# pearsonlab/autoencoded-vocal-analysis

Hardware: AMD Instinct MI355X
Metric: spectrograms/sec, VAE train step (fwd+bwd+Adam), 128x128, batch 256 per GPU (higher is better)
Workload: dtype f32 (fc1/fc8 products, the forward convolutions with >= 8 input channels and the fused backward kernels (data gradient AND weight gradient): fp32 operands as three bf16 limbs on bf16 MFMA, six limb products, fp32 accumulate; the 1<->8-channel layers, convt6's forward, conv7's forward and the small f; 1 GPU; configs[1]: mouse_sylls VAE, batch 256 synthetic 128x128 fp32 spectrograms per GPU, z=32, train step = zero_grad+forward+backward+Adam, device-resident batches; global_batch=256, per_gpu_batch=256, z_dim=32, parallelism=dp1

## Files before the change

autoencoded-vocal-analysis_amd/_lib.py:

```python
import ctypes as C
import os
import subprocess

_HERE = os.path.dirname(os.path.abspath(__file__))
CSRC = os.path.join(_HERE, "csrc")
_TAG = os.environ.get("AVA_HIP_LIB_TAG", "")
LIB_PATH = os.path.join(CSRC, "libava_hip_%s.so" % _TAG if _TAG else "libava_hip.so")

_ERR = {-1: "AVA_EINVAL (bad argument / unsupported shape)", -2: "AVA_ELAUNCH (HIP launch failure)",
        -3: "AVA_EWORKSPACE (workspace too small)"}


class AvaHipError(RuntimeError):
    pass


def build(force=False, verbose=False):
    cmd = ["make", "-C", CSRC, "-j8"] + (["-B"] if force else [])
    res = subprocess.run(cmd, capture_output=True, text=True)
    if verbose or res.returncode != 0:
        print(res.stdout)
        print(res.stderr)
    if res.returncode != 0:
        raise AvaHipError("building libava_hip.so failed")
    return LIB_PATH


_p = C.c_void_p
_i = C.c_int
_i64 = C.c_int64
_f = C.c_float
_d = C.c_double
_sz = C.c_size_t

SIGNATURES = {
    "ava_version": (_i, []),
    "ava_arena_floats": (_i64, [_i]),
    "ava_param_offset": (_i64, [_i, _i, C.POINTER(_i64)]),
    "ava_workspace_bytes": (_sz, [_i, _i]),
    "ava_model_create": (_i, [C.POINTER(_p), _i, _i, _f, _p, _p, _p, _p, _p, _p, _p, _sz]),
    "ava_model_destroy": (None, [_p]),
    "ava_arena_floats_hw": (_i64, [_i, _i, _i]),
    "ava_param_offset_hw": (_i64, [_i, _i, _i, _i, C.POINTER(_i64)]),
    "ava_workspace_bytes_hw": (_sz, [_i, _i, _i, _i]),
    "ava_model_create_hw": (_i, [C.POINTER(_p), _i, _i, _i, _i, _f, _p, _p, _p, _p, _p, _p, _p, _sz]),
    "ava_model_create_ex": (_i, [C.POINTER(_p), _i, _i, _i, _i, _i, _f, _p, _p, _p, _p, _p, _p, _p, _sz]),
    "ava_forward": (_i, [_p, _p, _i, _p, _p, _i, _p, _p, _p, _p]),
    "ava_forward_noise": (_i, [_p, _p, _i, _p, C.c_uint64, C.c_uint64, _i, _p, _p, _p, _p]),
    "ava_backward": (_i, [_p, _p, _i, _p]),
    "ava_set_backward_scale": (_i, [_p, _p]),
    "ava_backward_num_parts": (_i, []),
    "ava_backward_part": (_i, [_p, _p, _i, _i, _p]),
    "ava_grad_bucket": (_i, [_p, _i, C.POINTER(_i64), C.POINTER(_i64)]),
    "ava_adam_step": (_i, [_p, _d, _d, _d, _d, _i, _p]),
    "ava_adam_step_range": (_i, [_p, _i64, _i64, _d, _d, _d, _d, _i, _p]),
    "ava_encode": (_i, [_p, _p, _i, _i, _p, _p, _p, _p]),
    "ava_decode": (_i, [_p, _p, _i, _i, _p, _p]),
    "ava_last_z": (_p, [_p]),
    "ava_last_xrec": (_p, [_p]),
    "ava_debug_buffer": (_p, [_p, C.c_char_p, C.POINTER(_i64)]),
    "ava_debug_materialize": (_i, [_p, _p, _i, _p]),
    "ava_set_cu_reserve": (_i, [_i]),
    "ava_get_cu_reserve": (_i, []),
    "ava_model_set_cu_reserve": (_i, [_p, _i]),
    "ava_model_get_cu_reserve": (_i, [_p]),
    "ava_occupy_cus": (_i, [_i, _i, _f, _p]),
    "ava_profile_enable": (_i, [_p, _i]),
    "ava_profile_read": (_i, [_p, C.POINTER(_f), C.POINTER(_i)]),
    "ava_fill_normal": (_i, [_p, _i64, C.c_uint64, C.c_uint64, _p]),
    "ava_pack_conv_weight": (_i, [_p, _p, _i, _i, _i, _p]),
    "ava_conv_grid": (_i, [_i, _i, _i, _i]),
    "ava_conv3x3": (_i, [_p] * 13 + [_i] * 9 + [_f, _p]),
    "ava_conv3x3_wgrad": (_i, [_p] * 9 + [_i] * 7 + [_p]),
    "ava_conv_wgrad_grid": (_i, [_i, _i, _i, _i]),
    "ava_conv_wgrad_rows": (_i, [_i, _i, _i, _i, _i, _i, _i]),
    "ava_conv_fused_grid": (_i, [_i, _i, _i, _i, _i, _i]),
    "ava_conv3x3_bwd_fused": (_i, [_p] * 14 + [_i] * 7 + [_p]),
    "ava_conv_wgrad_reduce": (_i, [_p, _i, _p, _p, _i, _i, _i, _p]),
    "ava_bn_stats": (_i, [_p, _i64, _i, _p, C.POINTER(_i), _p]),
    "ava_bn_finalize": (_i, [_p, _i, _i64, _i, _p, _p, _p, _p, _p, _i, _p, _p, _p, _p, _p]),
    "ava_bn_finalize_bwd": (_i, [_p, _i, _i64, _i, _p, _p, _p, _p, _p, _p, _p, _p, _p]),
    "ava_gemm_workspace_bytes": (_sz, [_i, _i, _i]),
    "ava_gemm": (_i, [_p, _i, _p, _i, _p, _p, _i, _p, _p, _i, _i, _i, _i, _i, _i, _p, _sz, _p]),
    "ava_latent_fwd": (_i, [_p] * 9 + [_i, _i, _p]),
    "ava_latent_bwd": (_i, [_p] * 9 + [_i, _i, _p]),
    "ava_elbo_finalize": (_i, [_p, _i, _p, _i, _i, _f, _p, _p]),
    "ava_adam_flat": (_i, [_p, _p, _p, _p, _i64, _d, _d, _d, _d, _i, _p]),
    "ava_cast_to_f32": (_i, [_p, _i, _i64, _p, _p]),
    "ava_host_gather_rows": (_i, [_p, _p, _p, _i64, _i64, _sz, _i]),
    "ava_mmd2_workspace_bytes": (_sz, [_i, _i]),
    "ava_mmd2": (_i, [_p, _i, _p, _i, _p, _i, _d, _p, _p, _sz, _p]),
    "ava_mmd2_linear": (_i, [_p, _i, _p, _p, _i, _d, _p, _p, _sz, _p]),
    "ava_pair_sqdist": (_i, [_p, _i, _p, _p, _i, _p, _p]),
    "ava_spec_workspace_bytes": (_sz, [_i, _i, _i, _i, _i, _i, _i]),
    "ava_get_spec_batch": (_i, [_p, _i, _p, _p, _p, _p, _p, _p, _i, _i, _d, _i, _i, _p, _d, _p, _i, _i, _d, _d, _d, _i,
                                _i, _i, _d, _p, _p, _p, _sz, _p]),
    "ava_amp_workspace_bytes": (_sz, [_i64]),
    "ava_amp_trace": (_i, [_p, _i, _p, _p, _p, _i, _i64, _i, _i, _p, _d, _i, _i, _d, _d, _i, _d, _p, _i, _i, _p, _p, _p,
                           _sz, _p]),
    "ava_amp_decide": (_i, [_p, _i, _p, _i, _i64, _d, _d, _d, _p, _p, _p, _p, _i64, _p]),
    "ava_tpl_workspace_bytes": (_sz, [_i64]),
    "ava_tpl_tile_lags": (_i, []),
    "ava_tpl_spec": (_i, [_p, _i, _p, _p, _p, _i, _i64, _i, _i, _p, _d, _i, _i, _d, _d, _p, _p, _p]),
    "ava_tpl_xcorr": (_i, [_p, _p, _i, _i64, _p, _p, _p, _i, _i64, _i64, _p, _i, _i, _p, _p, _sz, _p]),
    "ava_warp_cache_bytes": (_sz, [_i, _d, _d, _i, _i, _d, _d]),
    "ava_warp_cache_layout": (_i, [_i, _d, _d, _i, _i, _d, _d, C.POINTER(_i64)]),
    "ava_warp_cache_workspace_bytes": (_sz, [_i, _d, _d, _i, _i]),
    "ava_warp_cache_build": (_i, [_p, _i, _p, _p, _i, _d, _d, _i, _i, _p, _d, _d, _d, _i, _p, _sz, _p, _sz, _p]),
    "ava_warp_windows_workspace_bytes": (_sz, [_i, _i, _i, _i]),
    "ava_warp_windows": (_i, [_p, _sz, _i, _d, _d, _i, _i, _d, _d, _p, _p, _i, _p, _i, _i, _d, _d, _d, _i, _i, _d, _p, _p,
                              _sz, _p]),
    "ava_warp_band_spec": (_i, [_p, _i, _p, _p, _p, _i, _i64, _i, _i, _p, _d, _i, _i, _d, _d, _p, _p, _p]),
    "ava_nn_workspace_bytes": (_sz, [_i, _i, _i, _i]),
    "ava_nn_argmin": (_i, [_p, _i, _i, _p, _i, _i, _i, _i, _p, _p, _p, _sz, _p]),
    "ava_nn_merge": (_i, [_p, _p, _p, _p, _i, _i64, _i, _p]),
    "ava_pj_knn": (_i, [_p, _i, _i, _i, _i, _i, _i, _p, _p, _p]),
    "ava_pj_smooth": (_i, [_p, _p, _i, _i, _d, _p, _p, _p, _p, _p]),
    "ava_pj_layout": (_i, [_p, _p, _p, _p, _p, _p, _p, _p, _i, _i64, _i, _i, _i, _d, _d, _d, _d, C.c_uint64, _p, _p]),
    "ava_pj_gram_workspace_bytes": (_sz, [_i, _i]),
    "ava_pj_gram": (_i, [_p, _i, _i, _i, _p, _p, _sz, _p]),
    "ava_pj_project": (_i, [_p, _i, _i, _i, _p, _p, _i, _p, _p]),
}

_lib = None


def load():
    global _lib
    if _lib is not None:
        return _lib
    if not os.path.exists(LIB_PATH):
        raise AvaHipError(
            "%s not found: the HIP extension is the only backend of this package. Build it with "
            "`python -c 'import __graft_entry__ as g; g.build()'` or `make -C %s`." % (LIB_PATH, CSRC))
    import torch
    lib = C.CDLL(LIB_PATH)
    for name, (res, args) in SIGNATURES.items():
        fn = getattr(lib, name)
        fn.restype = res
        fn.argtypes = args
    _lib = lib
    return lib


def check(rc, what):
    if rc != 0:
        raise AvaHipError("%s failed: %s" % (what, _ERR.get(rc, rc)))


def ptr(t):
    return None if t is None else t.data_ptr()


def stream():
    import torch
    return torch.cuda.current_stream().cuda_stream
```

autoencoded-vocal-analysis_amd/csrc/gemm.h:

```cpp
#pragma once
#include "common.h"

enum { ACT_NONE = 0, ACT_RELU = 1, ACT_EXP = 2 };

struct GemmArgs {
  const float* A;
  const float* B;
  const float* bias;
  float* C;
  float* colsum;
  const float* mask;
  int M, N, K;
  int lda, ldb, ldc;
  int klen;
  int splits;
  int act;
  int vec_a, vec_b;
};

#ifdef __HIPCC__
__device__ __forceinline__ float apply_act(float v, int act) {
  if (act == ACT_RELU) return fmaxf(v, 0.f);
  if (act == ACT_EXP) return expf(v);
  return v;
}
#endif

bool ava_gemm_limb_ok(const GemmArgs& g, int a_kmajor, int b_kmajor);
void ava_gemm_limb_plan(int M, int N, int K, int a_kmajor, int* bn, int* splits, int* klen);
int ava_gemm_limb_launch(const GemmArgs& g, int a_kmajor, int b_kmajor, int bn, hipStream_t st);
```

autoencoded-vocal-analysis_amd/csrc/gemm.hip:

```cpp
#include <stdlib.h>
#include "gemm.h"

typedef float f32x16 __attribute__((ext_vector_type(16)));

#define AVA_OPAQUE4(v) asm volatile("" : "+v"((v).x), "+v"((v).y), "+v"((v).z), "+v"((v).w))

template <int BT, int BK, bool KMAJ, bool VEC>
struct OperandLoader {
  static constexpr int N = BT * BK / 4 / 256;
  float4 r[N];
  int off[N];
  unsigned okrow;
  unsigned okk;
  int kk[N];

  __device__ __forceinline__ void init(int t0, int extent, int ld) {
    okrow = 0u;
#pragma unroll
    for (int i = 0; i < N; ++i) {
      const int v = threadIdx.x + 256 * i;
      if (KMAJ) {
        const int row = v / (BK / 4), kq = v % (BK / 4);
        const int g = t0 + row;
        if (g < extent) okrow |= 1u << i;
        off[i] = min(g, extent - 1) * ld;
        kk[i] = 4 * kq;
      } else {
        const int k = v / (BT / 4), m4 = v % (BT / 4);
        const int g = t0 + 4 * m4;
        if (g < extent) okrow |= 1u << i;
        off[i] = VEC ? min(g, extent - 4) : g;
        kk[i] = k;
      }
    }
  }

  __device__ __forceinline__ void load(const float* __restrict__ base, int ld, int extent, int k0, int kend, int K) {
    okk = VEC ? 0u : 0xffffffffu;
#pragma unroll
    for (int i = 0; i < N; ++i) {
      float4 x;
      if (KMAJ) {
        const int gk = k0 + kk[i];
        if (VEC) {
          x = *reinterpret_cast<const float4*>(base + off[i] + min(gk, K - 4));
          if (gk < kend) okk |= 1u << i;
        } else {
          const float* p = base + off[i];
          const bool ok = (okrow >> i) & 1u;
          x.x = (ok && gk + 0 < kend) ? p[min(gk + 0, K - 1)] : 0.f;
          x.y = (ok && gk + 1 < kend) ? p[min(gk + 1, K - 1)] : 0.f;
          x.z = (ok && gk + 2 < kend) ? p[min(gk + 2, K - 1)] : 0.f;
          x.w = (ok && gk + 3 < kend) ? p[min(gk + 3, K - 1)] : 0.f;
        }
      } else {
        const int gk = k0 + kk[i];
        const float* p = base + (size_t)min(gk, K - 1) * ld;
        if (VEC) {
          x = *reinterpret_cast<const float4*>(p + off[i]);
          if (gk < kend) okk |= 1u << i;
        } else {
          const int g = off[i];
          const bool okk = gk < kend;
          x.x = (okk && g + 0 < extent) ? p[min(g + 0, extent - 1)] : 0.f;
          x.y = (okk && g + 1 < extent) ? p[min(g + 1, extent - 1)] : 0.f;
          x.z = (okk && g + 2 < extent) ? p[min(g + 2, extent - 1)] : 0.f;
          x.w = (okk && g + 3 < extent) ? p[min(g + 3, extent - 1)] : 0.f;
        }
      }
      r[i] = x;
    }
  }

  template <int LD>
  __device__ __forceinline__ void store(float* __restrict__ S) const {
#pragma unroll
    for (int i = 0; i < N; ++i) {
      const int v = threadIdx.x + 256 * i;
      float4 x = r[i];
      if (VEC && !((okrow & okk) >> i & 1u)) x = make_float4(0.f, 0.f, 0.f, 0.f);
      if (KMAJ) {
        const int row = v / (BK / 4), kq = v % (BK / 4);
        S[(4 * kq + 0) * LD + row] = x.x;
        S[(4 * kq + 1) * LD + row] = x.y;
        S[(4 * kq + 2) * LD + row] = x.z;
        S[(4 * kq + 3) * LD + row] = x.w;
      } else {
        const int k = v / (BT / 4), m4 = v % (BT / 4);
        *reinterpret_cast<float4*>(&S[k * LD + 4 * m4]) = x;
      }
    }
  }
};

template <int BM, int BN, bool A_KMAJ, bool B_KMAJ, int BK, bool VEC>
__device__ __forceinline__ void gemm_body(const GemmArgs& g, const int bx, const int by, const int split) {
  constexpr int LDA_S = BM + (A_KMAJ ? 2 : 4);
  constexpr int LDB_S = BN + (B_KMAJ ? 2 : 4);
  constexpr int WM = BM / 2, WN = BN / 2;
  constexpr int TM = WM / 32, TN = WN / 32;
  constexpr int LDC_S = BN + 4;
  constexpr int OPER_F = 2 * BK * LDA_S + 2 * BK * LDB_S, CT_F = BM * LDC_S;
  __shared__ __align__(16) float smem_all[OPER_F > CT_F ? OPER_F : CT_F];
  float (*As2)[BK * LDA_S] = reinterpret_cast<float (*)[BK * LDA_S]>(smem_all);
  float (*Bs2)[BK * LDB_S] = reinterpret_cast<float (*)[BK * LDB_S]>(smem_all + 2 * BK * LDA_S);

  const int t = threadIdx.x, lane = t & 63, wave = t >> 6;
  const int wm = wave >> 1, wn = wave & 1;
  const int m0 = by * BM, n0 = bx * BN;
  const int kbeg = split * g.klen;
  const int kend = min(g.K, kbeg + g.klen);

  f32x16 acc[TM][TN];
#pragma unroll
  for (int i = 0; i < TM; ++i)
#pragma unroll
    for (int j = 0; j < TN; ++j)
#pragma unroll
      for (int r = 0; r < 16; ++r) acc[i][j][r] = 0.f;

  OperandLoader<BM, BK, A_KMAJ, VEC> la;
  OperandLoader<BN, BK, B_KMAJ, VEC> lb;
  la.init(m0, g.M, g.lda);
  lb.init(n0, g.N, g.ldb);

  float csum = 0.f;
  const bool do_colsum = g.colsum != nullptr && bx == 0;

  const int kq = lane >> 5, li = lane & 31;
  if (kbeg < kend) {
    la.load(g.A, g.lda, g.M, kbeg, kend, g.K);
    lb.load(g.B, g.ldb, g.N, kbeg, kend, g.K);
    la.template store<LDA_S>(As2[0]);
    lb.template store<LDB_S>(Bs2[0]);
    la.load(g.A, g.lda, g.M, kbeg + BK, kend, g.K);
    lb.load(g.B, g.ldb, g.N, kbeg + BK, kend, g.K);
  }
  __syncthreads();
  int cur = 0;
  for (int k0 = kbeg; k0 < kend; k0 += BK) {
    const float* As = As2[cur];
    const float* Bs = Bs2[cur];
    if (do_colsum && t < BM) {
#pragma unroll
      for (int k = 0; k < BK; ++k) csum += As[k * LDA_S + t];
    }
    float af[2][TM], bf[2][TN];
#pragma unroll
    for (int i = 0; i < TM; ++i) af[0][i] = As[kq * LDA_S + wm * WM + i * 32 + li];
#pragma unroll
    for (int j = 0; j < TN; ++j) bf[0][j] = Bs[kq * LDB_S + wn * WN + j * 32 + li];
#pragma unroll
    for (int kk = 0; kk < BK; kk += 2) {
      const int c = (kk >> 1) & 1, nx = c ^ 1;
      if (kk + 2 < BK) {
#pragma unroll
        for (int i = 0; i < TM; ++i) af[nx][i] = As[(kk + 2 + kq) * LDA_S + wm * WM + i * 32 + li];
#pragma unroll
        for (int j = 0; j < TN; ++j) bf[nx][j] = Bs[(kk + 2 + kq) * LDB_S + wn * WN + j * 32 + li];
      }
#pragma unroll
      for (int i = 0; i < TM; ++i)
#pragma unroll
        for (int j = 0; j < TN; ++j)
          acc[i][j] = __builtin_amdgcn_mfma_f32_32x32x2f32(af[c][i], bf[c][j], acc[i][j], 0, 0, 0);
      if (kk == BK / 2 - 2) {
        la.template store<LDA_S>(As2[cur ^ 1]);
        lb.template store<LDB_S>(Bs2[cur ^ 1]);
        la.load(g.A, g.lda, g.M, k0 + 2 * BK, kend, g.K);
        lb.load(g.B, g.ldb, g.N, k0 + 2 * BK, kend, g.K);
      }
    }
    __syncthreads();
    cur ^= 1;
  }

  float* Ct = smem_all;
#pragma unroll
  for (int i = 0; i < TM; ++i)
#pragma unroll
    for (int j = 0; j < TN; ++j)
#pragma unroll
      for (int r = 0; r < 16; ++r) {
        const int row = wm * WM + i * 32 + (r & 3) + 8 * (r >> 2) + 4 * (lane >> 5);
        Ct[row * LDC_S + wn * WN + j * 32 + (lane & 31)] = acc[i][j][r];
      }
  __syncthreads();
  float* Cout = g.C + (size_t)split * g.M * g.N;
  const bool fin = g.splits == 1;
  const int ldo = fin ? g.ldc : g.N;
  float* __restrict__ obase = fin ? g.C : Cout;
  constexpr int QPR = BN / 4;
  const bool vec_out = (ldo % 4 == 0) && ((reinterpret_cast<uintptr_t>(obase) & 15) == 0) && (n0 + BN <= g.N) &&
                       (!fin || g.mask == nullptr || ((reinterpret_cast<uintptr_t>(g.mask) & 15) == 0));
  for (int v = t; v < BM * QPR; v += 256) {
    const int row = v / QPR, q = v - row * QPR;
    const int gm = m0 + row, gn = n0 + 4 * q;
    if (gm >= g.M) continue;
    const float4 c4 = *reinterpret_cast<const float4*>(&Ct[row * LDC_S + 4 * q]);
    float cv[4] = {c4.x, c4.y, c4.z, c4.w};
    if (fin) {
#pragma unroll
      for (int e = 0; e < 4; ++e) {
        if (gn + e < g.N) {
          float x = cv[e] + (g.bias != nullptr ? g.bias[gn + e] : 0.f);
          x = apply_act(x, g.act);
          if (g.mask != nullptr && !(g.mask[(size_t)gm * g.ldc + gn + e] > 0.f)) x = 0.f;
          cv[e] = x;
        }
      }
    }
    float* dst = obase + (size_t)gm * ldo + gn;
    if (vec_out) {
      *reinterpret_cast<float4*>(dst) = make_float4(cv[0], cv[1], cv[2], cv[3]);
    } else {
#pragma unroll
      for (int e = 0; e < 4; ++e)
        if (gn + e < g.N) dst[e] = cv[e];
    }
  }
  if (do_colsum && t < BM && m0 + t < g.M) {
    if (fin) g.colsum[m0 + t] = csum;
    else g.C[(size_t)g.splits * g.M * g.N + (size_t)split * g.M + m0 + t] = csum;
  }
}

template <int BM, int BN, bool A_KMAJ, bool B_KMAJ, int BK, bool VEC>
__global__ __launch_bounds__(256) void gemm_kernel(const GemmArgs g) {
  gemm_body<BM, BN, A_KMAJ, B_KMAJ, BK, VEC>(g, blockIdx.x, blockIdx.y, blockIdx.z);
}

#define AVA_GEMM_GROUP_MAX 8
struct GemmGroup {
  GemmArgs g[AVA_GEMM_GROUP_MAX];
  int tile0[AVA_GEMM_GROUP_MAX + 1];
  int n;
};
template <int BM, bool A_KMAJ, bool B_KMAJ, bool VEC>
__global__ __launch_bounds__(256) void gemm_grouped_kernel(const GemmGroup grp) {
  const GemmArgs& g = grp.g[blockIdx.z];
  if ((int)blockIdx.x * BM >= g.N || (int)blockIdx.y * BM >= g.M) return;
  gemm_body<BM, BM, A_KMAJ, B_KMAJ, 16, VEC>(g, blockIdx.x, blockIdx.y, 0);
}

__global__ void splitk_reduce_kernel(const float* __restrict__ ws, const float* __restrict__ bias,
                                     const float* __restrict__ mask, float* __restrict__ C,
                                     float* __restrict__ colsum, int M, int N, int ldc, int splits, int act) {
  const size_t mn = (size_t)M * N;
  if (colsum != nullptr && blockIdx.x == 0) {
    const float* cs = ws + (size_t)splits * mn;
    for (int m = threadIdx.x; m < M; m += blockDim.x) {
      float s = 0.f;
      for (int p = 0; p < splits; ++p) s += cs[(size_t)p * M + m];
      colsum[m] = s;
    }
  }
  for (size_t i = (size_t)blockIdx.x * blockDim.x + threadIdx.x; i < mn; i += (size_t)gridDim.x * blockDim.x) {
    float s = 0.f;
    int p = 0;
    for (; p + 8 <= splits; p += 8) {
      float v[8];
#pragma unroll
      for (int u = 0; u < 8; ++u) v[u] = ws[(size_t)(p + u) * mn + i];
#pragma unroll
      for (int u = 0; u < 8; ++u) s += v[u];
    }
    for (; p < splits; ++p) s += ws[(size_t)p * mn + i];
    const size_t m = i / N, n = i - m * N;
    if (bias != nullptr) s += bias[n];
    s = apply_act(s, act);
    if (mask != nullptr && !(mask[m * ldc + n] > 0.f)) s = 0.f;
    C[m * ldc + n] = s;
  }
}

typedef float f32x4g __attribute__((ext_vector_type(4)));

template <bool A_KMAJ, bool B_KMAJ>
__device__ __forceinline__ void gemm_skinny_body(const GemmArgs& g, const int bx, const int by) {
  __shared__ float red[7][64][4];
  __shared__ float cred[8][16];
  const int nw = blockDim.x >> 6;
  const int t = threadIdx.x, lane = t & 63, wave = t >> 6;
  const int i = lane & 15, kg = lane >> 4;
  const int m0 = by * 16, n0 = bx * 16;
  const int am = min(m0 + i, g.M - 1);
  const int bn = min(n0 + i, g.N - 1);
  const float* __restrict__ arow = A_KMAJ ? g.A + (size_t)am * g.lda : g.A + am;
  const float* __restrict__ bcol = B_KMAJ ? g.B + (size_t)bn * g.ldb : g.B + bn;
  const int nchunks = (g.K + 15) >> 4;
  const bool do_colsum = g.colsum != nullptr && bx == 0;
  f32x4g acc = {0.f, 0.f, 0.f, 0.f};
  float csum = 0.f;
  const int gn = n0 + i;
  float bv = 0.f, mk[4] = {1.f, 1.f, 1.f, 1.f};
  if (wave == 0 && gn < g.N) {
    if (g.bias != nullptr) bv = g.bias[gn];
    if (g.mask != nullptr) {
#pragma unroll
      for (int r = 0; r < 4; ++r) mk[r] = g.mask[(size_t)min(m0 + 4 * kg + r, g.M - 1) * g.ldc + gn];
    }
  }
  constexpr int U = 4;
  for (int c0 = wave; c0 < nchunks; c0 += nw * U) {
    f32x4g a[U], b[U];
#pragma unroll
    for (int u = 0; u < U; ++u) {
      const int k = 16 * (c0 + nw * u) + 4 * kg;
      if (A_KMAJ) {
        const bool ok = k < g.K;
        a[u] = *reinterpret_cast<const f32x4g*>(arow + (ok ? k : 0));
        if (!ok) a[u] = (f32x4g){0.f, 0.f, 0.f, 0.f};
      } else {
#pragma unroll
        for (int j = 0; j < 4; ++j) {
          const float v = arow[(size_t)min(k + j, g.K - 1) * g.lda];
          a[u][j] = k + j < g.K ? v : 0.f;
        }
      }
      if (B_KMAJ) {
        b[u] = *reinterpret_cast<const f32x4g*>(bcol + (k < g.K ? k : 0));
      } else {
#pragma unroll
        for (int j = 0; j < 4; ++j) b[u][j] = bcol[(size_t)min(k + j, g.K - 1) * g.ldb];
      }
    }
#pragma unroll
    for (int u = 0; u < U; ++u)
#pragma unroll
      for (int j = 0; j < 4; ++j) {
        acc = __builtin_amdgcn_mfma_f32_16x16x4f32(a[u][j], b[u][j], acc, 0, 0, 0);
        csum += a[u][j];
      }
  }
  if (wave > 0) {
#pragma unroll
    for (int r = 0; r < 4; ++r) red[wave - 1][lane][r] = acc[r];
  }
  if (do_colsum) {
    csum += __shfl_xor(csum, 16, 64);
    csum += __shfl_xor(csum, 32, 64);
    if (kg == 0) cred[wave][i] = csum;
  }
  __syncthreads();
  if (wave != 0) return;
  if (do_colsum && kg == 0 && m0 + i < g.M) {
    float cs = cred[0][i];
    for (int w = 1; w < nw; ++w) cs += cred[w][i];
    g.colsum[m0 + i] = cs;
  }
  if (gn >= g.N) return;
#pragma unroll
  for (int r = 0; r < 4; ++r) {
    const int gm = m0 + 4 * kg + r;
    if (gm < g.M) {
      float v = acc[r];
      for (int w = 0; w + 1 < nw; ++w) v += red[w][lane][r];
      v = apply_act(v + bv, g.act);
      if (!(mk[r] > 0.f)) v = 0.f;
      g.C[(size_t)gm * g.ldc + gn] = v;
    }
  }
}

template <bool A_KMAJ, bool B_KMAJ>
__global__ __launch_bounds__(512) void gemm_skinny_kernel(const GemmArgs g) {
  gemm_skinny_body<A_KMAJ, B_KMAJ>(g, blockIdx.x, blockIdx.y);
}

static bool skinny_ok(const GemmArgs& g, int a_kmajor, int b_kmajor) {
  if (g.colsum != nullptr && a_kmajor) return false;
  if ((size_t)g.M * g.N > 262144 || g.K > 2048) return false;
  if (a_kmajor && (g.K % 4 != 0 || g.lda % 4 != 0 || (reinterpret_cast<uintptr_t>(g.A) & 15) != 0)) return false;
  if (b_kmajor && (g.K % 4 != 0 || g.ldb % 4 != 0 || (reinterpret_cast<uintptr_t>(g.B) & 15) != 0)) return false;
  return true;
}

template <bool A_KMAJ, bool B_KMAJ>
__global__ __launch_bounds__(512) void gemm_skinny_grouped_kernel(const GemmGroup grp) {
  int p = 0;
  while (p + 1 < grp.n && (int)blockIdx.x >= grp.tile0[p + 1]) ++p;
  const GemmArgs& g = grp.g[p];
  const int tile = blockIdx.x - grp.tile0[p], tx = (g.N + 15) >> 4;
  gemm_skinny_body<A_KMAJ, B_KMAJ>(g, tile % tx, tile / tx);
}

static void plan(int M, int N, int K, int* bm, int* splits, int* klen) {
  *bm = (M >= 128 && N >= 128) ? 128 : 64;
  if ((size_t)M * N <= 262144 && K <= 2048) *bm = 64;
  const bool wide = M <= 256 && K >= 512 && ceil_div(M, 64) * ceil_div(N, 64) >= 384;
  const bool deep = M <= 256 && K >= 4096 && (size_t)M * N <= 262144;
  if (wide || deep) *bm = 64;
  const int tiles = ceil_div(M, *bm) * ceil_div(N, *bm);
  int s = 1;
  if (tiles < 384) {
    s = ceil_div(deep ? 1024 : 512, tiles);
    const int max_s = K / 32 > 0 ? K / 32 : 1;
    if (s > max_s) s = max_s;
    if (s < 1) s = 1;
  }
  int kl = ceil_div(ceil_div(K, s), 16) * 16;
  s = ceil_div(K, kl);
  *splits = s;
  *klen = kl;
}

extern "C" size_t ava_gemm_workspace_bytes(int M, int N, int K) {
  int bm, splits, klen;
  plan(M, N, K, &bm, &splits, &klen);
  int lbn, lsplits, lklen;
  for (int ak = 0; ak < 2; ++ak) {
    ava_gemm_limb_plan(M, N, K, ak, &lbn, &lsplits, &lklen);
    if (lsplits > splits) splits = lsplits;
  }
  return splits > 1 ? ((size_t)splits * M * N + (size_t)splits * M) * sizeof(float) : 0;
}

template <int BM, int BK, bool VEC>
static void launch_gemm(const GemmArgs& g, int a_k, int b_k, dim3 grid, hipStream_t st) {
  if (a_k && b_k) hipLaunchKernelGGL((gemm_kernel<BM, BM, true, true, BK, VEC>), grid, dim3(256), 0, st, g);
  else if (a_k && !b_k) hipLaunchKernelGGL((gemm_kernel<BM, BM, true, false, BK, VEC>), grid, dim3(256), 0, st, g);
  else if (!a_k && b_k) hipLaunchKernelGGL((gemm_kernel<BM, BM, false, true, BK, VEC>), grid, dim3(256), 0, st, g);
  else hipLaunchKernelGGL((gemm_kernel<BM, BM, false, false, BK, VEC>), grid, dim3(256), 0, st, g);
}

static int gemm_impl(const float* A, int lda, const float* B, int ldb, const float* bias, float* C, int ldc,
                     const float* mask, float* colsum, int M, int N, int K, int a_kmajor, int b_kmajor, int act,
                     void* ws, size_t ws_bytes, ava_stream_t s, int* deferred_slabs);

extern "C" int ava_gemm(const float* A, int lda, const float* B, int ldb, const float* bias, float* C, int ldc,
                        const float* mask, float* colsum, int M, int N, int K, int a_kmajor, int b_kmajor, int act,
                        void* ws, size_t ws_bytes, ava_stream_t s) {
  return gemm_impl(A, lda, B, ldb, bias, C, ldc, mask, colsum, M, N, K, a_kmajor, b_kmajor, act, ws, ws_bytes, s, nullptr);
}

int ava_gemm_defer2(const float* A, int lda, const float* B, int ldb, const float* bias, float* C, int ldc,
                    const float* mask, float* colsum, int M, int N, int K, int a_kmajor, int b_kmajor, int act,
                    void* ws, size_t ws_bytes, ava_stream_t s, int* slabs) {
  *slabs = 1;
  return gemm_impl(A, lda, B, ldb, bias, C, ldc, mask, colsum, M, N, K, a_kmajor, b_kmajor, act, ws, ws_bytes, s, slabs);
}

static int gemm_impl(const float* A, int lda, const float* B, int ldb, const float* bias, float* C, int ldc,
                     const float* mask, float* colsum, int M, int N, int K, int a_kmajor, int b_kmajor, int act,
                     void* ws, size_t ws_bytes, ava_stream_t s, int* deferred_slabs) {
  if (A == nullptr || B == nullptr || C == nullptr || M <= 0 || N <= 0 || K <= 0) return AVA_EINVAL;
  int bm, splits, klen;
  plan(M, N, K, &bm, &splits, &klen);
  if (splits > 1 && (ws == nullptr || ws_bytes < ava_gemm_workspace_bytes(M, N, K))) return AVA_EWORKSPACE;
  GemmArgs g;
  g.A = A; g.B = B; g.bias = bias; g.colsum = colsum; g.mask = mask;
  g.C = splits > 1 ? reinterpret_cast<float*>(ws) : C;
  g.M = M; g.N = N; g.K = K;
  g.lda = lda > 0 ? lda : (a_kmajor ? K : M);
  g.ldb = ldb > 0 ? ldb : (b_kmajor ? K : N);
  g.ldc = ldc > 0 ? ldc : N;
  g.klen = klen; g.splits = splits; g.act = act;
  g.vec_a = (g.lda % 4 == 0) && ((reinterpret_cast<uintptr_t>(A) & 15) == 0) && (a_kmajor ? K % 4 == 0 && K >= 4 : M % 4 == 0 && M >= 4);
  g.vec_b = (g.ldb % 4 == 0) && ((reinterpret_cast<uintptr_t>(B) & 15) == 0) && (b_kmajor ? K % 4 == 0 && K >= 4 : N % 4 == 0 && N >= 4);
  const bool vec = g.vec_a && g.vec_b;
  hipStream_t st = to_stream(s);
  if (ava_gemm_limb_ok(g, a_kmajor, b_kmajor)) {
    int lbn;
    ava_gemm_limb_plan(M, N, K, a_kmajor, &lbn, &splits, &klen);
    if (splits > 1 && (ws == nullptr || ws_bytes < ((size_t)splits * M * N + (size_t)splits * M) * sizeof(float)))
      return AVA_EWORKSPACE;
    g.klen = klen; g.splits = splits;
    g.C = splits > 1 ? reinterpret_cast<float*>(ws) : C;
    const int rc = ava_gemm_limb_launch(g, a_kmajor, b_kmajor, lbn, st);
    if (rc != AVA_OK) return rc;
    if (splits == 2 && deferred_slabs != nullptr && mask == nullptr && colsum == nullptr && g.ldc == N) {
      *deferred_slabs = 2;
      return AVA_OK;
    }
    if (splits > 1) {
      const size_t mn = (size_t)M * N;
      int blocks = (int)((mn + 255) / 256);
      if (blocks > 2048) blocks = 2048;
      hipLaunchKernelGGL(splitk_reduce_kernel, dim3(blocks), dim3(256), 0, st, reinterpret_cast<const float*>(ws), bias,
                         mask, C, colsum, M, N, g.ldc, splits, act);
      AVA_CHECK_LAUNCH();
    }
    return AVA_OK;
  }
  if (skinny_ok(g, a_kmajor, b_kmajor)) {
    g.C = C;
    const dim3 sgrid(ceil_div(N, 16), ceil_div(M, 16));
    const dim3 sblock(K >= 512 ? 512 : 256);
    if (a_kmajor && b_kmajor) hipLaunchKernelGGL((gemm_skinny_kernel<true, true>), sgrid, sblock, 0, st, g);
    else if (a_kmajor) hipLaunchKernelGGL((gemm_skinny_kernel<true, false>), sgrid, sblock, 0, st, g);
    else if (b_kmajor) hipLaunchKernelGGL((gemm_skinny_kernel<false, true>), sgrid, sblock, 0, st, g);
    else hipLaunchKernelGGL((gemm_skinny_kernel<false, false>), sgrid, sblock, 0, st, g);
    AVA_CHECK_LAUNCH();
    return AVA_OK;
  }
  dim3 grid(ceil_div(N, bm), ceil_div(M, bm), splits);
  if (!vec) {
    if (bm == 128) launch_gemm<128, 16, false>(g, a_kmajor, b_kmajor, grid, st);
    else launch_gemm<64, 16, false>(g, a_kmajor, b_kmajor, grid, st);
  } else if (bm == 128) {
    if (klen % 32 == 0) launch_gemm<128, 32, true>(g, a_kmajor, b_kmajor, grid, st);
    else launch_gemm<128, 16, true>(g, a_kmajor, b_kmajor, grid, st);
  } else {
    if (klen % 32 == 0 && klen >= 512) launch_gemm<64, 32, true>(g, a_kmajor, b_kmajor, grid, st);
    else launch_gemm<64, 16, true>(g, a_kmajor, b_kmajor, grid, st);
  }
  AVA_CHECK_LAUNCH();
  if (splits > 1) {
    const size_t mn = (size_t)M * N;
    int blocks = (int)((mn + 255) / 256);
    if (blocks > 2048) blocks = 2048;
    hipLaunchKernelGGL(splitk_reduce_kernel, dim3(blocks), dim3(256), 0, st, reinterpret_cast<const float*>(ws), bias,
                       mask, C, colsum, M, N, g.ldc, splits, act);
    AVA_CHECK_LAUNCH();
  }
  return AVA_OK;
}

struct AvaGemmProblem {
  const float* A; int lda; const float* B; int ldb; const float* bias; float* C; int ldc; const float* mask;
  float* colsum; int M, N, K; int act;
};
int ava_gemm_grouped(const AvaGemmProblem* p, int n, int a_kmajor, int b_kmajor, hipStream_t st) {
  if (n < 1 || n > AVA_GEMM_GROUP_MAX) return AVA_EINVAL;
  GemmGroup grp;
  bool vec = true;
  int tx = 1, ty = 1;
  for (int i = 0; i < n; ++i) {
    GemmArgs& g = grp.g[i];
    if (p[i].A == nullptr || p[i].B == nullptr || p[i].C == nullptr || p[i].M <= 0 || p[i].N <= 0 || p[i].K <= 0)
      return AVA_EINVAL;
    g.A = p[i].A; g.B = p[i].B; g.bias = p[i].bias; g.C = p[i].C; g.colsum = p[i].colsum; g.mask = p[i].mask;
    g.M = p[i].M; g.N = p[i].N; g.K = p[i].K;
    g.lda = p[i].lda > 0 ? p[i].lda : (a_kmajor ? g.K : g.M);
    g.ldb = p[i].ldb > 0 ? p[i].ldb : (b_kmajor ? g.K : g.N);
    g.ldc = p[i].ldc > 0 ? p[i].ldc : g.N;
    g.klen = ceil_div(g.K, 16) * 16; g.splits = 1; g.act = p[i].act;
    g.vec_a = (g.lda % 4 == 0) && ((reinterpret_cast<uintptr_t>(g.A) & 15) == 0) &&
              (a_kmajor ? g.K % 4 == 0 && g.K >= 4 : g.M % 4 == 0 && g.M >= 4);
    g.vec_b = (g.ldb % 4 == 0) && ((reinterpret_cast<uintptr_t>(g.B) & 15) == 0) &&
              (b_kmajor ? g.K % 4 == 0 && g.K >= 4 : g.N % 4 == 0 && g.N >= 4);
    vec = vec && g.vec_a && g.vec_b;
    tx = tx > ceil_div(g.N, 64) ? tx : ceil_div(g.N, 64);
    ty = ty > ceil_div(g.M, 64) ? ty : ceil_div(g.M, 64);
  }
  bool skinny = true;
  int tiles = 0;
  for (int i = 0; i < n; ++i) {
    skinny = skinny && skinny_ok(grp.g[i], a_kmajor, b_kmajor);
    grp.tile0[i] = tiles;
    tiles += ceil_div(grp.g[i].N, 16) * ceil_div(grp.g[i].M, 16);
  }
  grp.tile0[n] = tiles;
  grp.n = n;
  if (skinny) {
    const dim3 sgrid(tiles);
    if (a_kmajor && b_kmajor) hipLaunchKernelGGL((gemm_skinny_grouped_kernel<true, true>), sgrid, dim3(256), 0, st, grp);
    else if (a_kmajor) hipLaunchKernelGGL((gemm_skinny_grouped_kernel<true, false>), sgrid, dim3(256), 0, st, grp);
    else if (b_kmajor) hipLaunchKernelGGL((gemm_skinny_grouped_kernel<false, true>), sgrid, dim3(256), 0, st, grp);
    else hipLaunchKernelGGL((gemm_skinny_grouped_kernel<false, false>), sgrid, dim3(256), 0, st, grp);
    AVA_CHECK_LAUNCH();
    return AVA_OK;
  }
  const dim3 grid(tx, ty, n);
#define AVA_GG(AK, BK_)                                                                                          \
  if (vec) hipLaunchKernelGGL((gemm_grouped_kernel<64, AK, BK_, true>), grid, dim3(256), 0, st, grp);            \
  else hipLaunchKernelGGL((gemm_grouped_kernel<64, AK, BK_, false>), grid, dim3(256), 0, st, grp);
  if (a_kmajor && b_kmajor) { AVA_GG(true, true) }
  else if (a_kmajor && !b_kmajor) { AVA_GG(true, false) }
  else if (!a_kmajor && b_kmajor) { AVA_GG(false, true) }
  else { AVA_GG(false, false) }
#undef AVA_GG
  AVA_CHECK_LAUNCH();
  return AVA_OK;
}
```

autoencoded-vocal-analysis_amd/csrc/gemm_limb.hip:

```cpp
#include <type_traits>
#include "gemm.h"

typedef __bf16 bf16x8 __attribute__((ext_vector_type(8)));
typedef __bf16 bf16x2 __attribute__((ext_vector_type(2)));
typedef float f32x2 __attribute__((ext_vector_type(2)));
typedef float f32x4 __attribute__((ext_vector_type(4)));
typedef uint32_t u32x4 __attribute__((ext_vector_type(4)));
typedef uint32_t u32x2 __attribute__((ext_vector_type(2)));

#define LBK 32

__device__ __forceinline__ float limb_sub(float a, float b) {
  float r;
  asm("v_sub_f32 %0, %1, %2" : "=v"(r) : "v"(a), "v"(b));
  return r;
}
__device__ __forceinline__ void limb_split2(float x, float y, uint32_t& p0, uint32_t& p1, uint32_t& p2) {
  p0 = __builtin_bit_cast(uint32_t, __builtin_convertvector((f32x2){x, y}, bf16x2));
  float rx = limb_sub(x, __uint_as_float(p0 << 16)), ry = limb_sub(y, __uint_as_float(p0 & 0xffff0000u));
  p1 = __builtin_bit_cast(uint32_t, __builtin_convertvector((f32x2){rx, ry}, bf16x2));
  rx = limb_sub(rx, __uint_as_float(p1 << 16));
  ry = limb_sub(ry, __uint_as_float(p1 & 0xffff0000u));
  p2 = __builtin_bit_cast(uint32_t, __builtin_convertvector((f32x2){rx, ry}, bf16x2));
}

template <bool PERM>
__device__ __forceinline__ int pos16(int r) {
  return PERM ? ((r & ~5) | ((r & 1) << 2) | ((r >> 2) & 1)) : r;
}
template <bool PERM>
__device__ __forceinline__ int chunk_of(int r, int oct) {
  return PERM ? (oct ^ ((r & 1) << 1)) : (oct ^ ((4 - ((r >> 2) & 3)) & 3));
}


template <int BT, int T, int LIMB_RING>
struct LimbLoaderK {
  static constexpr int UNITS = BT * 4, NU = (UNITS + T - 1) / T;
  float4 r[LIMB_RING][NU][2];
  unsigned ok[LIMB_RING];
  size_t off[NU];
  unsigned okrow;
  __device__ __forceinline__ void init(int t0, int extent, int ld) {
    okrow = 0u;
#pragma unroll
    for (int i = 0; i < NU; ++i) {
      const int u = threadIdx.x + T * i, row = u >> 2, oct = u & 3, g = t0 + row;
      if (u < UNITS && g < extent) okrow |= 1u << i;
      off[i] = (size_t)min(g, extent - 1) * ld + oct * 8;
    }
  }
  template <int SLOT>
  __device__ __forceinline__ void load(const float* __restrict__ base, int , int k0, int kend, int K) {
    unsigned okk = 0u;
#pragma unroll
    for (int i = 0; i < NU; ++i) {
      const int oct = (threadIdx.x + T * i) & 3, gk = k0 + oct * 8;
      const float* p = base + off[i] + min(k0, K - 8 - oct * 8);
      r[SLOT][i][0] = *reinterpret_cast<const float4*>(p);
      r[SLOT][i][1] = *reinterpret_cast<const float4*>(p + 4);
      if (gk < kend) okk |= 1u << i;
    }
    ok[SLOT] = okk & okrow;
  }
  template <int SLOT, bool COLSUM>
  __device__ __forceinline__ void store(unsigned char* __restrict__ S) {
#pragma unroll
    for (int i = 0; i < NU; ++i) {
      const int u = threadIdx.x + T * i, row = u >> 2, oct = u & 3;
      if (UNITS % T != 0 && u >= UNITS) continue;
      float4 a = r[SLOT][i][0], b = r[SLOT][i][1];
      if (!((ok[SLOT] >> i) & 1u)) { a = make_float4(0.f, 0.f, 0.f, 0.f); b = a; }
      u32x4 p0, p1, p2;
      uint32_t x, y, z;
      limb_split2(a.x, a.y, x, y, z); p0[0] = x; p1[0] = y; p2[0] = z;
      limb_split2(a.z, a.w, x, y, z); p0[1] = x; p1[1] = y; p2[1] = z;
      limb_split2(b.x, b.y, x, y, z); p0[2] = x; p1[2] = y; p2[2] = z;
      limb_split2(b.z, b.w, x, y, z); p0[3] = x; p1[3] = y; p2[3] = z;
      unsigned char* d = S + row * 64 + chunk_of<false>(row & 15, oct) * 16;
      *reinterpret_cast<u32x4*>(d) = p0;
      *reinterpret_cast<u32x4*>(d + BT * 64) = p1;
      *reinterpret_cast<u32x4*>(d + 2 * BT * 64) = p2;
    }
  }
};

template <int BT, int T, int LIMB_RING>
struct LimbLoaderN {
  static constexpr int KPU = (2 * BT >= T) ? 4 : 2;
  static constexpr int KQ = LBK / KPU;
  static constexpr int UNITS = (BT / 4) * KQ, NU = (UNITS + T - 1) / T;
  float4 r[LIMB_RING][NU][KPU];
  unsigned ok[LIMB_RING];
  int coff[NU];
  unsigned okcol;
  float cs[NU][4];
  __device__ __forceinline__ LimbLoaderN() {
#pragma unroll
    for (int i = 0; i < NU; ++i)
#pragma unroll
      for (int c = 0; c < 4; ++c) cs[i][c] = 0.f;
  }
  __device__ __forceinline__ void init(int t0, int extent, int ) {
    okcol = 0u;
#pragma unroll
    for (int i = 0; i < NU; ++i) {
      const int u = threadIdx.x + T * i, cq = u / KQ, g = t0 + 4 * cq;
      if (u < UNITS && g < extent) okcol |= ((1u << KPU) - 1u) << (KPU * i);
      coff[i] = min(g, extent - 4);
    }
  }
  template <int SLOT>
  __device__ __forceinline__ void load(const float* __restrict__ base, int ld, int k0, int kend, int K) {
    unsigned okk = 0u;
#pragma unroll
    for (int i = 0; i < NU; ++i) {
      const int kq = (threadIdx.x + T * i) % KQ;
#pragma unroll
      for (int j = 0; j < KPU; ++j) {
        const int gk = k0 + KPU * kq + j;
        r[SLOT][i][j] = *reinterpret_cast<const float4*>(base + (size_t)min(gk, K - 1) * ld + coff[i]);
        if (gk < kend) okk |= 1u << (KPU * i + j);
      }
    }
    ok[SLOT] = okk & okcol;
  }
  template <int SLOT, bool COLSUM>
  __device__ __forceinline__ void store(unsigned char* __restrict__ S) {
#pragma unroll
    for (int i = 0; i < NU; ++i) {
      const int u = threadIdx.x + T * i, kq = u % KQ, cq = u / KQ;
      if (UNITS % T != 0 && u >= UNITS) continue;
      float v[KPU][4];
#pragma unroll
      for (int j = 0; j < KPU; ++j) {
        const bool okj = (ok[SLOT] >> (KPU * i + j)) & 1u;
        v[j][0] = okj ? r[SLOT][i][j].x : 0.f; v[j][1] = okj ? r[SLOT][i][j].y : 0.f;
        v[j][2] = okj ? r[SLOT][i][j].z : 0.f; v[j][3] = okj ? r[SLOT][i][j].w : 0.f;
      }
#pragma unroll
      for (int c = 0; c < 4; ++c) {
        const int row = 4 * cq + c;
        unsigned char* d = S + ((row & ~15) + pos16<true>(row & 15)) * 64;
        uint32_t x, y, z;
        if constexpr (KPU == 4) {
          if (COLSUM) cs[i][c] += (v[0][c] + v[1][c]) + (v[2][c] + v[3][c]);
          u32x2 p0, p1, p2;
          limb_split2(v[0][c], v[1][c], x, y, z); p0[0] = x; p1[0] = y; p2[0] = z;
          limb_split2(v[2][c], v[3][c], x, y, z); p0[1] = x; p1[1] = y; p2[1] = z;
          d += chunk_of<true>(row & 15, kq >> 1) * 16 + (kq & 1) * 8;
          *reinterpret_cast<u32x2*>(d) = p0;
          *reinterpret_cast<u32x2*>(d + BT * 64) = p1;
          *reinterpret_cast<u32x2*>(d + 2 * BT * 64) = p2;
        } else {
          if (COLSUM) cs[i][c] += v[0][c] + v[1][c];
          limb_split2(v[0][c], v[1][c], x, y, z);
          d += chunk_of<true>(row & 15, kq >> 2) * 16 + (kq & 3) * 4;
          *reinterpret_cast<uint32_t*>(d) = x;
          *reinterpret_cast<uint32_t*>(d + BT * 64) = y;
          *reinterpret_cast<uint32_t*>(d + 2 * BT * 64) = z;
        }
      }
    }
  }
};

template <int BT, int T, int RING, bool KMAJ>
struct LimbLoader;
template <int BT, int T, int RING>
struct LimbLoader<BT, T, RING, true> : LimbLoaderK<BT, T, RING> {};
template <int BT, int T, int RING>
struct LimbLoader<BT, T, RING, false> : LimbLoaderN<BT, T, RING> {};

template <int J, int R, class F>
__device__ __forceinline__ void limb_for_stage(F&& f) {
  f(std::integral_constant<int, J>{});
  if constexpr (J + 1 < R) limb_for_stage<J + 1, R>(f);
}

struct LimbItem { int m0, n0, split, kbeg, kend, bx; };

template <int BN, bool A_KMAJ, bool B_KMAJ, int RING, int MINW>
__global__ __launch_bounds__(512, MINW) void gemm_limb_kernel(const GemmArgs g, const int tiles_m, const int tiles_n,
                                                              const int nitems) {
  constexpr int NSW = 4;
  constexpr int BM = 128, T = 64 * NSW, WM = BM / 2, WN = BN / 2, TM = WM / 16, TN = WN / 16;
  constexpr int A_BYTES = 3 * BM * 64, B_BYTES = 3 * BN * 64, BUF = A_BYTES + B_BYTES;
  __shared__ __align__(16) unsigned char smem[2 * BUF];

  const int t = threadIdx.x, lane = t & 63, wave8 = t >> 6;
  const bool stager = wave8 < NSW;
  int it, it_end, it_step;
  {
    const int gsz = (int)gridDim.x, w = (int)blockIdx.x;
    if (((gsz | nitems) & 7) == 0) { const int chunk = nitems >> 3, x = w & 7; it = x * chunk + (w >> 3); it_end = (x + 1) * chunk; it_step = gsz >> 3; }
    else { it = w; it_end = nitems; it_step = gsz; }
  }
  auto decode = [&](int item) __attribute__((always_inline)) {
    LimbItem r;
    const int per = tiles_m * tiles_n;
    r.split = item / per;
    const int rem = item - r.split * per;
    const int by = rem / tiles_n;
    r.bx = rem - by * tiles_n;
    r.m0 = by * BM; r.n0 = r.bx * BN;
    r.kbeg = r.split * g.klen;
    r.kend = min(g.K, r.kbeg + g.klen);
    return r;
  };
  if (it >= it_end) return;

  if (stager) {
    __builtin_amdgcn_s_setprio(3);
    LimbLoader<BM, T, RING, A_KMAJ> la;
    LimbLoader<BN, T, RING, B_KMAJ> lb;
    int S = 0;
    for (int i = it; i < it_end; i += it_step) { const LimbItem q = decode(i); S += (q.kend - q.kbeg + LBK - 1) / LBK; }
    int l_it = it, s_it = it;
    LimbItem li = decode(l_it), si = li;
    int l_k = li.kbeg, s_k = si.kbeg;
    auto load_step = [&](auto slot) __attribute__((always_inline)) {
      constexpr int SLOT = decltype(slot)::value;
      if (l_k == li.kbeg) { la.init(li.m0, g.M, g.lda); lb.init(li.n0, g.N, g.ldb); }
      la.template load<SLOT>(g.A, g.lda, l_k, li.kend, g.K);
      lb.template load<SLOT>(g.B, g.ldb, l_k, li.kend, g.K);
      l_k += LBK;
      if (l_k >= li.kend) {
        l_it += it_step;
        if (l_it < it_end) { li = decode(l_it); l_k = li.kbeg; }
      }
    };
    auto store_step = [&](auto slot, int buf) __attribute__((always_inline)) {
      constexpr int SLOT = decltype(slot)::value;
      unsigned char* S_ = smem + buf * BUF;
      la.template store<SLOT, !A_KMAJ>(S_);
      lb.template store<SLOT, false>(S_ + A_BYTES);
      s_k += LBK;
      if (s_k >= si.kend) {
        if constexpr (!A_KMAJ) {
          if (g.colsum != nullptr && si.bx == 0) {
            const bool fin = g.splits == 1;
#pragma unroll
            for (int i = 0; i < LimbLoaderN<BM, T, RING>::NU; ++i) {
              constexpr int KQA = LimbLoaderN<BM, T, RING>::KQ;
              const int u = t + T * i, cq = u / KQA;
#pragma unroll
              for (int c = 0; c < 4; ++c) {
                float v = la.cs[i][c];
#pragma unroll
                for (int o = 1; o < KQA; o <<= 1) v += __shfl_xor(v, o, 64);
                const int gm = si.m0 + 4 * cq + c;
                if ((u % KQA) == 0 && u < LimbLoaderN<BM, T, RING>::UNITS && gm < g.M) {
                  if (fin) g.colsum[gm] = v;
                  else g.C[(size_t)g.splits * g.M * g.N + (size_t)si.split * g.M + gm] = v;
                }
              }
            }
          }
#pragma unroll
          for (int i = 0; i < LimbLoaderN<BM, T, RING>::NU; ++i)
#pragma unroll
            for (int c = 0; c < 4; ++c) la.cs[i][c] = 0.f;
        }
        s_it += it_step;
        if (s_it < it_end) { si = decode(s_it); s_k = si.kbeg; }
      }
    };
    limb_for_stage<0, RING - 1>([&](auto J) __attribute__((always_inline)) { if (decltype(J)::value < S) load_step(J); });
    store_step(std::integral_constant<int, 0>{}, 0);
    __syncthreads();
    int s0 = 0;
    for (; s0 + 2 * RING - 2 < S; s0 += RING)
      limb_for_stage<0, RING>([&](auto J) __attribute__((always_inline)) {
        constexpr int j = decltype(J)::value;
        load_step(std::integral_constant<int, (j + RING - 1) % RING>{});
        store_step(std::integral_constant<int, (j + 1) % RING>{}, (s0 + j + 1) & 1);
        __syncthreads();
      });
    for (; s0 < S; s0 += RING)
      limb_for_stage<0, RING>([&](auto J) __attribute__((always_inline)) {
        constexpr int j = decltype(J)::value;
        if (s0 + j < S) {
          if (s0 + j + RING - 1 < S) load_step(std::integral_constant<int, (j + RING - 1) % RING>{});
          if (s0 + j + 1 < S) store_step(std::integral_constant<int, (j + 1) % RING>{}, (s0 + j + 1) & 1);
          __syncthreads();
        }
      });
    return;
  }

  const int wave = wave8 - NSW, wm = wave >> 1, wn = wave & 1;
  const int fr = lane & 15, kg = lane >> 4;
  const int a_lane = (wm * WM) * 64 + pos16<!A_KMAJ>(fr) * 64 + chunk_of<!A_KMAJ>(fr, kg) * 16;
  const int b_lane = A_BYTES + (wn * WN) * 64 + pos16<!B_KMAJ>(fr) * 64 + chunk_of<!B_KMAJ>(fr, kg) * 16;
  f32x4 acc[TM][TN];
  __syncthreads();
  int s = 0;
  for (; it < it_end; it += it_step) {
    const LimbItem ci = decode(it);
#pragma unroll
    for (int i = 0; i < TM; ++i)
#pragma unroll
      for (int j = 0; j < TN; ++j) acc[i][j] = (f32x4){0.f, 0.f, 0.f, 0.f};
    for (int k0 = ci.kbeg; k0 < ci.kend; k0 += LBK, ++s) {
      const unsigned char* As = smem + (s & 1) * BUF + a_lane;
      const unsigned char* Bs = smem + (s & 1) * BUF + b_lane;
      bf16x8 af[TM][3];
#pragma unroll
      for (int i = 0; i < TM; ++i)
#pragma unroll
        for (int l = 0; l < 3; ++l) af[i][l] = *reinterpret_cast<const bf16x8*>(As + l * BM * 64 + i * 1024);
#pragma unroll
      for (int j = 0; j < TN; ++j) {
        bf16x8 bf[3];
#pragma unroll
        for (int l = 0; l < 3; ++l) bf[l] = *reinterpret_cast<const bf16x8*>(Bs + l * BN * 64 + j * 1024);
#pragma unroll
        for (int i = 0; i < TM; ++i) acc[i][j] = __builtin_amdgcn_mfma_f32_16x16x32_bf16(bf[0], af[i][2], acc[i][j], 0, 0, 0);
#pragma unroll
        for (int i = 0; i < TM; ++i) acc[i][j] = __builtin_amdgcn_mfma_f32_16x16x32_bf16(bf[2], af[i][0], acc[i][j], 0, 0, 0);
#pragma unroll
        for (int i = 0; i < TM; ++i) acc[i][j] = __builtin_amdgcn_mfma_f32_16x16x32_bf16(bf[1], af[i][1], acc[i][j], 0, 0, 0);
#pragma unroll
        for (int i = 0; i < TM; ++i) acc[i][j] = __builtin_amdgcn_mfma_f32_16x16x32_bf16(bf[0], af[i][1], acc[i][j], 0, 0, 0);
#pragma unroll
        for (int i = 0; i < TM; ++i) acc[i][j] = __builtin_amdgcn_mfma_f32_16x16x32_bf16(bf[1], af[i][0], acc[i][j], 0, 0, 0);
#pragma unroll
        for (int i = 0; i < TM; ++i) acc[i][j] = __builtin_amdgcn_mfma_f32_16x16x32_bf16(bf[0], af[i][0], acc[i][j], 0, 0, 0);
      }
      __syncthreads();
    }
    const bool fin = g.splits == 1;
    const int ldo = fin ? g.ldc : g.N;
    float* __restrict__ obase = fin ? g.C : g.C + (size_t)ci.split * g.M * g.N;
    const bool plain = !fin || (g.bias == nullptr && g.mask == nullptr && g.act == ACT_NONE);
    const bool relu = g.act == ACT_RELU;
    if (plain) {
#pragma unroll
      for (int i = 0; i < TM; ++i) {
        const int gm = ci.m0 + wm * WM + i * 16 + fr;
        if (gm >= g.M) continue;
#pragma unroll
        for (int j = 0; j < TN; ++j) {
          const int gn = ci.n0 + wn * WN + j * 16 + 4 * kg;
          if (gn >= g.N) continue;
          *reinterpret_cast<f32x4*>(obase + (size_t)gm * ldo + gn) = acc[i][j];
        }
      }
    } else {
      float4 bq[TN];
#pragma unroll
      for (int j = 0; j < TN; ++j) {
        const int gn = ci.n0 + wn * WN + j * 16 + 4 * kg;
        bq[j] = make_float4(0.f, 0.f, 0.f, 0.f);
        if (g.bias != nullptr && gn < g.N) bq[j] = *reinterpret_cast<const float4*>(g.bias + gn);
      }
#pragma unroll
      for (int i = 0; i < TM; ++i) {
        const int gm = ci.m0 + wm * WM + i * 16 + fr;
        if (gm >= g.M) continue;
#pragma unroll
        for (int j = 0; j < TN; ++j) {
          const int gn = ci.n0 + wn * WN + j * 16 + 4 * kg;
          if (gn >= g.N) continue;
          float cv[4] = {acc[i][j][0], acc[i][j][1], acc[i][j][2], acc[i][j][3]};
          cv[0] += bq[j].x; cv[1] += bq[j].y; cv[2] += bq[j].z; cv[3] += bq[j].w;
          if (relu) { cv[0] = fmaxf(cv[0], 0.f); cv[1] = fmaxf(cv[1], 0.f); cv[2] = fmaxf(cv[2], 0.f); cv[3] = fmaxf(cv[3], 0.f); }
          if (g.mask != nullptr) {
            const float4 mk = *reinterpret_cast<const float4*>(g.mask + (size_t)gm * g.ldc + gn);
            if (!(mk.x > 0.f)) cv[0] = 0.f;
            if (!(mk.y > 0.f)) cv[1] = 0.f;
            if (!(mk.z > 0.f)) cv[2] = 0.f;
            if (!(mk.w > 0.f)) cv[3] = 0.f;
          }
          *reinterpret_cast<float4*>(obase + (size_t)gm * ldo + gn) = make_float4(cv[0], cv[1], cv[2], cv[3]);
        }
      }
    }
  }
}

static bool limb_shape(int M, int N, int K) {
  const int mn = M < N ? M : N, mnk = mn < K ? mn : K;
  const size_t pair = (size_t)M * N * K / (size_t)mnk;
  return pair >= ((size_t)1 << 22);
}

bool ava_gemm_limb_ok(const GemmArgs& g, int a_kmajor, int b_kmajor) {
  if (!limb_shape(g.M, g.N, g.K) || !g.vec_a || !g.vec_b) return false;
  if ((a_kmajor || b_kmajor) && g.K % 8 != 0) return false;
  if (!a_kmajor && g.M % 4 != 0) return false;
  if (!b_kmajor && g.N % 4 != 0) return false;
  if (g.colsum != nullptr && a_kmajor) return false;
  if (g.act != ACT_NONE && g.act != ACT_RELU) return false;
  if (g.N % 4 != 0 || g.ldc % 4 != 0 || (reinterpret_cast<uintptr_t>(g.C) & 15) != 0) return false;
  if (g.bias != nullptr && (reinterpret_cast<uintptr_t>(g.bias) & 15) != 0) return false;
  if (g.mask != nullptr && (reinterpret_cast<uintptr_t>(g.mask) & 15) != 0) return false;
  return true;
}

void ava_gemm_limb_plan(int M, int N, int K, int a_kmajor, int* bn, int* splits, int* klen) {
  const int b = a_kmajor ? 64 : 128;
  const int tiles = ceil_div(M, 128) * ceil_div(N, b);
  const int want = b == 64 ? 512 : 256;
  int s = 1;
  if (tiles < want * 3 / 4) {
    s = ceil_div(want, tiles);
    const int max_s = K / 64 > 0 ? K / 64 : 1;
    if (s > max_s) s = max_s;
  }
  int kl = ceil_div(ceil_div(K, s), LBK) * LBK;
  s = ceil_div(K, kl);
  *bn = b; *splits = s; *klen = kl;
}

int ava_gemm_limb_launch(const GemmArgs& g, int a_kmajor, int b_kmajor, int bn, hipStream_t st) {
  const int tm = ceil_div(g.M, 128), tn = ceil_div(g.N, bn), nitems = tm * tn * g.splits;
  static int cus = 0;
  if (cus == 0) {
    int dev = 0;
    hipDeviceProp_t prop;
    cus = (hipGetDevice(&dev) == hipSuccess && hipGetDeviceProperties(&prop, dev) == hipSuccess && prop.multiProcessorCount > 0)
              ? prop.multiProcessorCount : 256;
  }
  const int resident = ava_scale_grid((bn == 64 ? 2 : 1) * cus);
  int grid = nitems < resident ? nitems : resident;
  if (bn == 64 && a_kmajor) {
    if (b_kmajor) hipLaunchKernelGGL((gemm_limb_kernel<64, true, true, 3, 4>), dim3(grid), dim3(512), 0, st, g, tm, tn, nitems);
    else hipLaunchKernelGGL((gemm_limb_kernel<64, true, false, 3, 4>), dim3(grid), dim3(512), 0, st, g, tm, tn, nitems);
  } else if (bn == 128 && !a_kmajor) {
    if (b_kmajor) hipLaunchKernelGGL((gemm_limb_kernel<128, false, true, 4, 2>), dim3(grid), dim3(512), 0, st, g, tm, tn, nitems);
    else hipLaunchKernelGGL((gemm_limb_kernel<128, false, false, 4, 2>), dim3(grid), dim3(512), 0, st, g, tm, tn, nitems);
  }
  else return AVA_EINVAL;
  AVA_CHECK_LAUNCH();
  return AVA_OK;
}
```

autoencoded-vocal-analysis_amd/csrc/model.hip:

```cpp
#include <stdlib.h>
#include <string.h>
#include <string>
#include <map>
#include "conv_common.h"
#include "conv_fused.h"

int ava_nchw_to_nhwc_stats(const float* in, float* out, float* partials, int B, int P, int act_bf16, long long* acc_out,
                           int* nparts, hipStream_t st);
int ava_conv3x3_wgrad_ex(const float* x, const float* xa, const float* xb, const float* dy, const float* dy2,
                         const float* da, const float* db_, const float* dc, float* partials, int B, int Hi, int Wi,
                         int Cin, int Cout, int mode, int dy_pro, int act_bf16, ava_stream_t s);
int ava_conv_wgrad_rows_ex(int B, int Hi, int Wi, int Cin, int Cout, int mode, int dy_pro, int act_bf16);
int ava_bn_eval_all(const float* const* gamma, const float* const* beta, const int* C, const float* running, float* save,
                    hipStream_t st);
int ava_conv3x3_ex(const float* in, const float* in2, const float* pa, const float* pb, const float* pc,
                   const float* G, const float* bias, float* out, float* out2, const float* epi_x,
                   const float* epi_mean, const float* epi_invstd, float* partials, int B, int Hi, int Wi, int Cin,
                   int Cout, int mode, int pro, int epi, int relu, float prec, int act_bf16, const ConvAcc* acc, ava_stream_t s);
int ava_nhwc_to_nchw(const float* in, float* out, int B, int P, hipStream_t st);
int ava_relu_mask_to_nhwc(const float* dy_nchw, const float* slab1, const float* y_nhwc, float* du, int B, int P, hipStream_t st);
int ava_nchw_to_nhwc_stats_slabs(const float* slab0, const float* slab1, const float* bias, int relu, float* full, float* out,
                                 float* partials, int B, int P, int act_bf16, long long* acc_out, int* nparts, hipStream_t st);
int ava_gemm_defer2(const float* A, int lda, const float* B, int ldb, const float* bias, float* C, int ldc,
                    const float* mask, float* colsum, int M, int N, int K, int a_kmajor, int b_kmajor, int act,
                    void* ws, size_t ws_bytes, ava_stream_t s, int* slabs);
int ava_bn_bwd_apply_to_nchw(const float* g, const float* f8, const float* A, const float* Bc, const float* Cc,
                             float* out, int B, int P, int act_bf16, const BnFin* fin, hipStream_t st);
int ava_bn_finalize_bwd_ex(const float* partials, int nparts, int64_t n, int C, const float* gamma, const float* mean,
                           const float* invstd, float* dgamma, float* dbeta, float* A, float* Bc, float* Cc, int eval,
                           hipStream_t st);
int ava_scale_backward_roots(float* seed, int64_t n, float* wg, int64_t nwg, long long* slot, const float* scale, hipStream_t st);
int ava_adam_flat_guarded(float* p, const float* g, float* m, float* v, int64_t n, double lr, double beta1, double beta2,
                          double eps, int step, const int* skip_if_set, hipStream_t st);
int ava_elbo_finalize_strided(const float* latent_sums, int B, const float* sse_partials, int nparts, int stride,
                              int zdim, float prec, int xdim, float* loss_out, double* loss_accum, hipStream_t st);

enum { ACT_NONE = 0, ACT_RELU = 1, ACT_EXP = 2 };

struct FcMidFwdArgs {
  const float* h3_in;
  const float *W3, *b3;
  const float *W41, *b41, *W42, *b42, *W43, *b43;
  const float *W5, *b5, *W6, *b6;
  const float *eps_w, *eps_d;
  float *h3, *mu, *u, *logd, *d, *z, *lat_sums, *h5, *h6;
  int* status;
  int B, zdim;
};
struct FcMidBwdArgs {
  const float* dh6;
  const float *W6, *W5, *W41, *W42, *W43, *W3;
  const float *h5, *h3, *h2;
  const float *z, *u, *d, *eps_w, *eps_d;
  const float* scale;
  float *dh5, *dz, *dmu, *du, *dlogd, *dh3, *dh2;
  int B, zdim;
};
int ava_fc_mid_fwd(const FcMidFwdArgs& a, hipStream_t st);
int ava_fc_mid_bwd(const FcMidBwdArgs& a, hipStream_t st);

#define NCONV 14
#define NPARAM 80
#define ALIGN_F 64

enum { CAT_CONV_FWD = 0, CAT_CONV_BWD_DATA, CAT_CONV_WGRAD, CAT_BN, CAT_GEMM, CAT_LAYOUT, CAT_LATENT_LOSS, CAT_ADAM,
       CAT_PACK, NCAT };
#define PROF_MAX_EVENTS 1024
struct Prof {
  bool on = false;
  int mode = 0;
  int n = 0;
  hipEvent_t ev[PROF_MAX_EVENTS];
  int cat[PROF_MAX_EVENTS];
  int created = 0;
  int seq_fam[PROF_MAX_EVENTS];
  int seq_n = 0;
  int idx = 0;
};
static inline int prof_family(int cat) {
  if (cat < 0) return -1;
  return (cat == CAT_CONV_FWD || cat == CAT_CONV_BWD_DATA || cat == CAT_CONV_WGRAD || cat == CAT_BN || cat == CAT_PACK) ? 0 : 1;
}

struct ConvLayer {
  int cin, cout, mode;
  int hi, ho;
  int transposed;
  int pw, pb, pg, pbeta;
};
struct LayerDims { int hi, wi, ho, wo; };

static const ConvLayer kLayers[NCONV] = {
    {1, 8, MODE_S1, 128, 128, 0, 0, 1, 14, 15},    {8, 8, MODE_DOWN, 128, 64, 0, 2, 3, 16, 17},
    {8, 16, MODE_S1, 64, 64, 0, 4, 5, 18, 19},     {16, 16, MODE_DOWN, 64, 32, 0, 6, 7, 20, 21},
    {16, 24, MODE_S1, 32, 32, 0, 8, 9, 22, 23},    {24, 24, MODE_DOWN, 32, 16, 0, 10, 11, 24, 25},
    {24, 32, MODE_S1, 16, 16, 0, 12, 13, 26, 27},  {32, 24, MODE_S1, 16, 16, 1, 52, 53, 66, 67},
    {24, 24, MODE_UP, 16, 32, 1, 54, 55, 68, 69},  {24, 16, MODE_S1, 32, 32, 1, 56, 57, 70, 71},
    {16, 16, MODE_UP, 32, 64, 1, 58, 59, 72, 73},  {16, 8, MODE_S1, 64, 64, 1, 60, 61, 74, 75},
    {8, 8, MODE_UP, 64, 128, 1, 62, 63, 76, 77},   {8, 1, MODE_S1, 128, 128, 1, 64, 65, 78, 79},
};

struct ParamInfo { int64_t off, numel; };

static void build_param_table(int z, int F, ParamInfo* tab, int64_t* total) {
  int64_t numel[NPARAM];
  int p = 0;
  const int enc[7][2] = {{1, 8}, {8, 8}, {8, 16}, {16, 16}, {16, 24}, {24, 24}, {24, 32}};
  for (int i = 0; i < 7; ++i) { numel[p++] = (int64_t)enc[i][0] * enc[i][1] * 9; numel[p++] = enc[i][1]; }
  const int bne[7] = {1, 8, 8, 16, 16, 24, 24};
  for (int i = 0; i < 7; ++i) { numel[p++] = bne[i]; numel[p++] = bne[i]; }
  const int fc[12][2] = {{F, 1024}, {1024, 256}, {256, 64}, {256, 64}, {256, 64}, {64, z}, {64, z}, {64, z},
                         {z, 64}, {64, 256}, {256, 1024}, {1024, F}};
  for (int i = 0; i < 12; ++i) { numel[p++] = (int64_t)fc[i][0] * fc[i][1]; numel[p++] = fc[i][1]; }
  const int dec[7][2] = {{32, 24}, {24, 24}, {24, 16}, {16, 16}, {16, 8}, {8, 8}, {8, 1}};
  for (int i = 0; i < 7; ++i) { numel[p++] = (int64_t)dec[i][0] * dec[i][1] * 9; numel[p++] = dec[i][1]; }
  const int bnd[7] = {32, 24, 24, 16, 16, 8, 8};
  for (int i = 0; i < 7; ++i) { numel[p++] = bnd[i]; numel[p++] = bnd[i]; }
  int order[NPARAM], n = 0;
  for (int i = 0; i < 32; ++i) order[n++] = i;
  order[n++] = 32; order[n++] = 34; order[n++] = 36;
  order[n++] = 33; order[n++] = 35; order[n++] = 37;
  for (int i = 38; i < NPARAM; ++i) order[n++] = i;
  int64_t cur = 0;
  for (int k = 0; k < NPARAM; ++k) {
    const int i = order[k];
    tab[i].off = cur;
    tab[i].numel = numel[i];
    cur += (numel[i] + ALIGN_F - 1) / ALIGN_F * ALIGN_F;
  }
  *total = cur;
}

struct ava_model {
  int z, maxB;
  int H, W;
  int P8, F;
  int act_bf16;
  LayerDims lay[NCONV];
  float prec;
  float *P, *G, *M, *V;
  float* bn_running;
  int64_t* bn_batches;
  ParamInfo tab[NPARAM];
  int64_t arena;
  float* X[NCONV];
  float *y7, *y7t;
  float *h1, *h2, *h3, *mu, *u, *logd, *d, *zs, *lat_sums;
  float *h5, *h6, *h7, *f8;
  float *xrec, *seed;
  float* bn_part;
  float* bn_save;
  float* bn_bwd;
  long long* bn_acc;
  int acc0_slot;
  int acc0_used;
  float* Gf[NCONV];
  float* Gb[NCONV];
  float *gA, *gB;
  int dy7_slabs;
  float* dy7_ws;
  size_t dy7_ws_bytes;
  int cu_reserve;
  float* wg_part[NCONV];
  float *dF8, *dh7, *dh6, *dh5, *dz, *dmu, *du, *dlogd, *dh3, *dh2, *dh1, *dy7;
  float* gemm_ws;
  size_t gemm_ws_bytes;
  float* loss_dev;
  int* status_dev;
  const float* eps_w_last;
  const float* eps_d_last;
  int sse_parts;
  int lastB;
  int last_train;
  int* status_last;
  const float* bwd_scale;
  int fold13;
  int wg13_rows;
  Prof prof;
  std::map<std::string, std::pair<const float*, int64_t>> dbg;
};

static inline float* bn_mean(ava_model* m, int l) { return m->bn_save + (l * 4 + 0) * 32; }
static inline float* bn_invstd(ava_model* m, int l) { return m->bn_save + (l * 4 + 1) * 32; }
static inline float* bn_scale(ava_model* m, int l) { return m->bn_save + (l * 4 + 2) * 32; }
static inline float* bn_shift(ava_model* m, int l) { return m->bn_save + (l * 4 + 3) * 32; }
static inline float* bn_A(ava_model* m, int l) { return m->bn_bwd + (l * 3 + 0) * 32; }
static inline float* bn_B(ava_model* m, int l) { return m->bn_bwd + (l * 3 + 1) * 32; }
static inline float* bn_C(ava_model* m, int l) { return m->bn_bwd + (l * 3 + 2) * 32; }
static inline float* PP(ava_model* m, int idx) { return m->P + m->tab[idx].off; }
static inline float* GG(ava_model* m, int idx) { return m->G + m->tab[idx].off; }

struct Carver {
  char* base;
  size_t off;
  float* take(size_t floats) {
    float* p = base ? reinterpret_cast<float*>(base + off) : nullptr;
    off += (floats * sizeof(float) + 255) / 256 * 256;
    return p;
  }
};

static size_t max_gemm_ws_at(int z, int B, int F) {
  size_t mx = 0;
  const int shapes[][3] = {{B, 1024, F}, {B, 256, 1024}, {B, 192, 256}, {B, z, 64}, {B, 64, z}, {B, 256, 64},
                           {B, 1024, 256}, {B, F, 1024},
                           {B, F, 1024}, {B, 1024, 256}, {B, 256, 192}, {B, 64, z}, {B, z, 64}, {B, 64, 256},
                           {B, 256, 1024}, {B, 1024, F},
                           {F, 1024, B}, {1024, 256, B}, {256, 64, B}, {64, z, B}, {z, 64, B}, {192, 256, B},
                           {256, 1024, B}, {1024, F, B}};
  for (auto& s : shapes) {
    size_t b = ava_gemm_workspace_bytes(s[0], s[1], s[2]);
    if (b > mx) mx = b;
  }
  return mx;
}
static size_t max_gemm_ws(int z, int maxB, int F) {
  size_t mx = 0;
  for (int b = 1; b <= maxB; ++b) { const size_t v = max_gemm_ws_at(z, b, F); if (v > mx) mx = v; }
  return mx;
}
static size_t max_dy7_ws(int maxB, int F) {
  size_t mx = 0;
  for (int b = 1; b <= maxB; ++b) { const size_t v = ava_gemm_workspace_bytes(b, F, 1024); if (v > mx) mx = v; }
  return mx;
}

static size_t wgrad_part_floats(const ava_model* m, int B, int l) {
  const ConvLayer& L = kLayers[l];
  const LayerDims& D = m->lay[l];
  int grid = ava_conv_wgrad_grid(B, D.ho, D.wo, L.mode);
  const int fg = ava_conv_fused_grid_for(B, D.hi, D.wi, L.cin, L.cout, L.mode);
  if (fg > grid) grid = fg;
  if (l == NCONV - 1) {
    const int fw = ava_conv_grid(B, D.ho, D.wo, L.mode);
    if (fw > grid) grid = fw;
  }
  return (size_t)grid * (9 * L.cin * L.cout + L.cout);
}

static void carve(ava_model* m, void* ws, size_t* total) {
  Carver c{reinterpret_cast<char*>(ws), 0};
  const size_t B = (size_t)m->maxB;
  const int z = m->z;
  const size_t F = (size_t)m->F, XD = (size_t)m->H * m->W;
  m->X[0] = nullptr;
  for (int l = 1; l < NCONV; ++l) {
    const ConvLayer& L = kLayers[l];
    if (l == 7) m->X[l] = c.take(B * F);
    else m->X[l] = c.take(B * m->lay[l].hi * m->lay[l].wi * L.cin);
  }
  m->y7 = c.take(B * F); m->y7t = c.take(B * F);
  m->h1 = c.take(B * 1024); m->h2 = c.take(B * 256); m->h3 = c.take(B * 192);
  m->mu = c.take(B * z); m->u = c.take(B * z); m->logd = c.take(B * z); m->d = c.take(B * z); m->zs = c.take(B * z);
  m->lat_sums = c.take(B * 2);
  m->h5 = c.take(B * 64); m->h6 = c.take(B * 256); m->h7 = c.take(B * 1024); m->f8 = c.take(B * F);
  m->xrec = c.take(B * XD); m->seed = c.take(B * XD);
  m->bn_part = c.take(1024 * 64);
  m->bn_save = c.take(NCONV * 4 * 32);
  m->bn_bwd = c.take(NCONV * 3 * 32);
  m->bn_acc = reinterpret_cast<long long*>(c.take((size_t)AVA_ACC_SLOTS * AVA_ACC_SLOT_LL * 2));
  for (int l = 0; l < NCONV; ++l) {
    m->Gf[l] = c.take(9 * kLayers[l].cin * kLayers[l].cout);
    m->Gb[l] = c.take(9 * kLayers[l].cin * kLayers[l].cout);
  }
  m->gA = c.take(B * XD * 8); m->gB = c.take(B * XD * 8);
  for (int l = 0; l < NCONV; ++l) m->wg_part[l] = c.take(wgrad_part_floats(m, (int)B, l));
  m->dF8 = c.take(B * F); m->dh7 = c.take(B * 1024); m->dh6 = c.take(B * 256); m->dh5 = c.take(B * 64);
  m->dz = c.take(B * z); m->dmu = c.take(B * z); m->du = c.take(B * z); m->dlogd = c.take(B * z);
  m->dh3 = c.take(B * 192); m->dh2 = c.take(B * 256); m->dh1 = c.take(B * 1024); m->dy7 = c.take(B * F);
  m->gemm_ws_bytes = max_gemm_ws(z, (int)B, m->F);
  m->gemm_ws = c.take(m->gemm_ws_bytes / sizeof(float) + 64);
  m->dy7_ws_bytes = max_dy7_ws((int)B, m->F);
  m->dy7_ws = c.take(m->dy7_ws_bytes / sizeof(float) + 64);
  m->loss_dev = c.take(64);
  m->status_dev = reinterpret_cast<int*>(c.take(64));
  *total = c.off;
}

extern "C" int ava_version(void) { return 100; }

static int g_cu_reserve_default = 0;
static thread_local int t_cu_reserve = -1;
int ava_cu_reserve(void) { return t_cu_reserve >= 0 ? t_cu_reserve : g_cu_reserve_default; }
extern "C" int ava_set_cu_reserve(int cus) {
  if (cus < 0 || cus > 128) return AVA_EINVAL;
  g_cu_reserve_default = cus;
  return AVA_OK;
}
extern "C" int ava_get_cu_reserve(void) { return g_cu_reserve_default; }
struct ReserveScope {
  int saved;
  explicit ReserveScope(const ava_model* m) : saved(t_cu_reserve) {
    if (m != nullptr) t_cu_reserve = m->cu_reserve >= 0 ? m->cu_reserve : g_cu_reserve_default;
  }
  ~ReserveScope() { t_cu_reserve = saved; }
};
extern "C" int ava_model_set_cu_reserve(ava_model* m, int cus) {
  if (m == nullptr || cus < -1 || cus > 128) return AVA_EINVAL;
  m->cu_reserve = cus;
  return AVA_OK;
}
extern "C" int ava_model_get_cu_reserve(const ava_model* m) { return m == nullptr ? -1 : m->cu_reserve; }

__global__ __launch_bounds__(256) void occupy_kernel(long long ticks, unsigned long long* sink) {
  extern __shared__ unsigned char occupy_lds[];
  if (ticks < 0) occupy_lds[threadIdx.x] = 0;
  const long long t0 = (long long)__builtin_amdgcn_s_memrealtime();
  long long n = 0;
  while ((long long)__builtin_amdgcn_s_memrealtime() - t0 < ticks) { __builtin_amdgcn_s_sleep(8); ++n; }
  if (sink != nullptr && threadIdx.x == 0 && blockIdx.x == 0) *sink = (unsigned long long)n;
}
extern "C" int ava_occupy_cus(int workgroups, int lds_bytes, float usec, ava_stream_t s) {
  if (workgroups < 1 || workgroups > 1024 || !(usec > 0.f) || usec > 20000.f || lds_bytes < 0 || lds_bytes > 160 * 1024)
    return AVA_EINVAL;
  static bool attr = false;
  if (!attr) {
    if (hipFuncSetAttribute(reinterpret_cast<const void*>(&occupy_kernel), hipFuncAttributeMaxDynamicSharedMemorySize,
                            160 * 1024) != hipSuccess) return AVA_ELAUNCH;
    attr = true;
  }
  hipLaunchKernelGGL(occupy_kernel, dim3(workgroups), dim3(256), (size_t)lds_bytes, to_stream(s), (long long)(usec * 100.f), nullptr);
  AVA_CHECK_LAUNCH();
  return AVA_OK;
}

static bool size_ok(int H, int W) { return (W == 128 || W == 256) && (H == 128 || H == 256); }

static void set_geometry(ava_model* m, int H, int W) {
  m->H = H; m->W = W;
  m->P8 = (H / 8) * (W / 8);
  m->F = 32 * m->P8;
  for (int l = 0; l < NCONV; ++l) {
    const ConvLayer& L = kLayers[l];
    m->lay[l].hi = L.hi * H / 128; m->lay[l].wi = L.hi * W / 128;
    m->lay[l].ho = L.ho * H / 128; m->lay[l].wo = L.ho * W / 128;
  }
}

extern "C" int64_t ava_arena_floats_hw(int z_dim, int H, int W) {
  if (!size_ok(H, W)) return -1;
  ParamInfo tab[NPARAM];
  int64_t total;
  build_param_table(z_dim, 32 * (H / 8) * (W / 8), tab, &total);
  return total;
}
extern "C" int64_t ava_param_offset_hw(int z_dim, int H, int W, int index, int64_t* numel) {
  if (index < 0 || index >= NPARAM || !size_ok(H, W)) return -1;
  ParamInfo tab[NPARAM];
  int64_t total;
  build_param_table(z_dim, 32 * (H / 8) * (W / 8), tab, &total);
  if (numel) *numel = tab[index].numel;
  return tab[index].off;
}
extern "C" size_t ava_workspace_bytes_hw(int z_dim, int H, int W, int max_batch) {
  if (!size_ok(H, W)) return 0;
  ava_model tmp;
  tmp.z = z_dim;
  tmp.maxB = max_batch;
  tmp.act_bf16 = 0;
  set_geometry(&tmp, H, W);
  size_t total = 0;
  carve(&tmp, nullptr, &total);
  return total;
}
extern "C" int64_t ava_arena_floats(int z_dim) { return ava_arena_floats_hw(z_dim, 128, 128); }
extern "C" int64_t ava_param_offset(int z_dim, int index, int64_t* numel) { return ava_param_offset_hw(z_dim, 128, 128, index, numel); }
extern "C" size_t ava_workspace_bytes(int z_dim, int max_batch) { return ava_workspace_bytes_hw(z_dim, 128, 128, max_batch); }

extern "C" int ava_model_create_ex(ava_model** out, int z_dim, int H, int W, int act_dtype, int max_batch,
                                   float model_precision, float* params, float* grads, float* exp_avg,
                                   float* exp_avg_sq, float* bn_running, int64_t* bn_batches, void* workspace,
                                   size_t workspace_bytes) {
  if (out == nullptr || z_dim < 1 || z_dim > 128 || max_batch < 1 || params == nullptr || workspace == nullptr ||
      !size_ok(H, W) || (act_dtype != 0 && act_dtype != 1))
    return AVA_EINVAL;
  ava_model* m = new ava_model();
  m->z = z_dim; m->maxB = max_batch; m->prec = model_precision;
  m->act_bf16 = act_dtype;
  set_geometry(m, H, W);
  m->P = params; m->G = grads; m->M = exp_avg; m->V = exp_avg_sq;
  m->bn_running = bn_running; m->bn_batches = bn_batches;
  build_param_table(z_dim, m->F, m->tab, &m->arena);
  size_t need = 0;
  carve(m, workspace, &need);
  if (need > workspace_bytes) { delete m; return AVA_EWORKSPACE; }
  m->lastB = 0;
  m->last_train = 1;
  m->cu_reserve = -1;
  m->dy7_slabs = 1;
  m->acc0_slot = -1; m->acc0_used = -1;
  m->status_last = nullptr;
  m->bwd_scale = nullptr;
  m->sse_parts = 0;
  m->fold13 = 0;
  m->wg13_rows = 0;
  const size_t B = max_batch;
  const int64_t F = m->F, XD = (int64_t)H * W;
  for (int l = 1; l < NCONV; ++l) {
    char nm[16];
    if (l < 7) { snprintf(nm, sizeof nm, "y%d", l); }
    else if (l == 7) { snprintf(nm, sizeof nm, "f8t"); }
    else { snprintf(nm, sizeof nm, "d%d", l - 7); }
    m->dbg[nm] = {m->X[l], (int64_t)(l == 7 ? B * F : B * m->lay[l].hi * m->lay[l].wi * kLayers[l].cin)};
  }
  m->dbg["y7"] = {m->y7, (int64_t)B * F}; m->dbg["y7t"] = {m->y7t, (int64_t)B * F};
  m->dbg["h1"] = {m->h1, (int64_t)B * 1024}; m->dbg["h2"] = {m->h2, (int64_t)B * 256};
  m->dbg["h3"] = {m->h3, (int64_t)B * 192};
  m->dbg["mu"] = {m->mu, (int64_t)B * z_dim}; m->dbg["u"] = {m->u, (int64_t)B * z_dim};
  m->dbg["logd"] = {m->logd, (int64_t)B * z_dim}; m->dbg["d"] = {m->d, (int64_t)B * z_dim};
  m->dbg["z"] = {m->zs, (int64_t)B * z_dim};
  m->dbg["h5"] = {m->h5, (int64_t)B * 64}; m->dbg["h6"] = {m->h6, (int64_t)B * 256};
  m->dbg["h7"] = {m->h7, (int64_t)B * 1024}; m->dbg["f8"] = {m->f8, (int64_t)B * F};
  m->dbg["xrec"] = {m->xrec, (int64_t)B * XD}; m->dbg["seed"] = {m->seed, (int64_t)B * XD};
  m->dbg["bn_save"] = {m->bn_save, NCONV * 4 * 32}; m->dbg["bn_bwd"] = {m->bn_bwd, NCONV * 3 * 32};
  m->dbg["dz"] = {m->dz, (int64_t)B * z_dim}; m->dbg["dF8"] = {m->dF8, (int64_t)B * F};
  m->dbg["wg13"] = {m->wg_part[NCONV - 1], (int64_t)wgrad_part_floats(m, (int)B, NCONV - 1)};
  *out = m;
  return AVA_OK;
}
extern "C" int ava_model_create_hw(ava_model** out, int z_dim, int H, int W, int max_batch, float model_precision,
                                   float* params, float* grads, float* exp_avg, float* exp_avg_sq, float* bn_running,
                                   int64_t* bn_batches, void* workspace, size_t workspace_bytes) {
  return ava_model_create_ex(out, z_dim, H, W, 0, max_batch, model_precision, params, grads, exp_avg, exp_avg_sq,
                             bn_running, bn_batches, workspace, workspace_bytes);
}
extern "C" int ava_model_create(ava_model** out, int z_dim, int max_batch, float model_precision, float* params,
                                float* grads, float* exp_avg, float* exp_avg_sq, float* bn_running,
                                int64_t* bn_batches, void* workspace, size_t workspace_bytes) {
  return ava_model_create_hw(out, z_dim, 128, 128, max_batch, model_precision, params, grads, exp_avg, exp_avg_sq,
                             bn_running, bn_batches, workspace, workspace_bytes);
}
extern "C" void ava_model_destroy(ava_model* m) { delete m; }
extern "C" const float* ava_last_z(ava_model* m) { return m->zs; }
extern "C" const float* ava_last_xrec(ava_model* m) { return m->xrec; }
extern "C" const float* ava_debug_buffer(ava_model* m, const char* name, int64_t* floats) {
  auto it = m->dbg.find(name);
  if (it == m->dbg.end()) return nullptr;
  if (floats) *floats = it->second.second;
  return it->second.first;
}

static inline void mark(ava_model* m, int cat, hipStream_t st) {
  Prof& p = m->prof;
  if (!p.on || p.n >= PROF_MAX_EVENTS) return;
  if (p.mode == 2) {
    const int i = p.idx++;
    const bool known = i < p.seq_n && p.seq_fam[i] == prof_family(cat);
    const bool boundary = !known || cat < 0 || i + 1 >= p.seq_n || p.seq_fam[i + 1] != p.seq_fam[i];
    if (!boundary) return;
  } else if (p.n < PROF_MAX_EVENTS) {
    p.seq_fam[p.n] = prof_family(cat);
  }
  if (p.n >= p.created) { if (hipEventCreate(&p.ev[p.created]) != hipSuccess) return; p.created++; }
  hipEventRecord(p.ev[p.n], st);
  p.cat[p.n] = cat;
  p.n++;
}

extern "C" int ava_profile_enable(ava_model* m, int on) {
  if (m == nullptr) return AVA_EINVAL;
  m->prof.on = on != 0;
  m->prof.mode = on == 2 ? 2 : 1;
  m->prof.n = 0;
  m->prof.idx = 0;
  return AVA_OK;
}
extern "C" int ava_profile_read(ava_model* m, float* ms, int* launches) {
  if (m == nullptr || ms == nullptr) return AVA_EINVAL;
  Prof& p = m->prof;
  if (p.n > 0) hipEventSynchronize(p.ev[p.n - 1]);
  for (int i = 1; i < p.n; ++i) {
    if (p.cat[i] < 0) continue;
    float e = 0.f;
    if (hipEventElapsedTime(&e, p.ev[i - 1], p.ev[i]) == hipSuccess) {
      ms[p.cat[i]] += e;
      if (launches) launches[p.cat[i]] += 1;
    }
  }
  if (p.mode == 1 && p.n > 0) p.seq_n = p.n;
  p.n = 0;
  p.idx = 0;
  return NCAT;
}

#define TRY(expr)            \
  do {                       \
    int _rc = (expr);        \
    if (_rc != AVA_OK) return _rc; \
  } while (0)

struct PackEntry { const float* w; float* g; int c0, c1, swap, flip; };
struct PackTable { PackEntry e[2 * NCONV]; long long* acc; int nacc; int keep0, keep1; long long* in_acc; };
__global__ void pack_all_kernel(const PackTable tab) {
  {
    const int gt = (blockIdx.y * gridDim.x + blockIdx.x) * blockDim.x + threadIdx.x, nt = gridDim.x * gridDim.y * blockDim.x;
    for (int i = gt; i < tab.nacc; i += nt) tab.acc[i] = 0;
  }
  const PackEntry e = tab.e[blockIdx.y];
  const int n = e.c0 * e.c1 * 9;
  for (int i = blockIdx.x * blockDim.x + threadIdx.x; i < n; i += gridDim.x * blockDim.x) {
    const int tt = i % 9, r = i / 9, i1 = r % e.c1, i0 = r / e.c1;
    const int tg = e.flip ? 8 - tt : tt;
    const int gi = e.swap ? (tg * e.c1 + i1) * e.c0 + i0 : (tg * e.c0 + i0) * e.c1 + i1;
    e.g[gi] = e.w[i];
  }
}
__global__ __launch_bounds__(256) void pack_stats_kernel(const PackTable tab, const float* __restrict__ x, int64_t n,
                                                         float* __restrict__ partials, int nstats, float* __restrict__ eps,
                                                         int64_t neps, uint64_t seed, uint64_t offset) {
  constexpr int NPACK = 7 * 2 * NCONV;
  for (int i = blockIdx.x * 256 + threadIdx.x; i < tab.nacc; i += gridDim.x * 256)
    if (i < tab.keep0 || i >= tab.keep1) tab.acc[i] = 0;
  if ((int)blockIdx.x >= nstats + NPACK) {
    const int nb = gridDim.x - nstats - NPACK, bi = blockIdx.x - nstats - NPACK;
    for (int64_t i = (int64_t)bi * 256 + threadIdx.x; i < neps; i += (int64_t)nb * 256)
      eps[i] = ava_normal_hash((uint64_t)i + offset, seed);
    return;
  }
  if ((int)blockIdx.x >= nstats) {
    const int idx = blockIdx.x - nstats, by = idx / 7, bx = idx - 7 * by;
    const PackEntry e = tab.e[by];
    const int cnt = e.c0 * e.c1 * 9;
    for (int i = bx * 256 + threadIdx.x; i < cnt; i += 7 * 256) {
      const int tt = i % 9, r = i / 9, i1 = r % e.c1, i0 = r / e.c1;
      const int tg = e.flip ? 8 - tt : tt;
      const int gi = e.swap ? (tg * e.c1 + i1) * e.c0 + i0 : (tg * e.c0 + i0) * e.c1 + i1;
      e.g[gi] = e.w[i];
    }
    return;
  }
  __shared__ float red[4][2];
  float s1 = 0.f, s2 = 0.f;
  const int64_t stride = (int64_t)nstats * 256, n4 = n / 4;
  const float4* x4 = reinterpret_cast<const float4*>(x);
  for (int64_t i = (int64_t)blockIdx.x * 256 + threadIdx.x; i < n4; i += stride) {
    const float4 v = x4[i];
    s1 += (v.x + v.y) + (v.z + v.w);
    s2 += (v.x * v.x + v.y * v.y) + (v.z * v.z + v.w * v.w);
  }
  if (blockIdx.x == 0 && threadIdx.x == 0)
    for (int64_t i = n4 * 4; i < n; ++i) { s1 += x[i]; s2 += x[i] * x[i]; }
  const int w = threadIdx.x >> 6, l = threadIdx.x & 63;
  const float r1 = wave_sum(s1), r2 = wave_sum(s2);
  if (l == 0) { red[w][0] = r1; red[w][1] = r2; }
  __syncthreads();
  if (threadIdx.x < 2) {
    const float tot = (red[0][threadIdx.x] + red[1][threadIdx.x]) + (red[2][threadIdx.x] + red[3][threadIdx.x]);
    if (tab.in_acc != nullptr) bn_acc_add(tab.in_acc, 32 * threadIdx.x, tot);
    else partials[(size_t)blockIdx.x * 2 + threadIdx.x] = tot;
  }
}

static long long* acc_slot(ava_model* m, int slot);
struct NoiseGen { float* eps; int64_t n; uint64_t seed, offset; };

static int pack_weights(ava_model* m, bool with_bwd, hipStream_t st, const float* x_stats = nullptr, int64_t n = 0,
                        int* nstats_out = nullptr, NoiseGen ng = NoiseGen{nullptr, 0, 0, 0}) {
  PackTable tab;
  for (int l = 0; l < NCONV; ++l) {
    const ConvLayer& L = kLayers[l];
    const float* w = PP(m, L.pw);
    const int c0 = L.transposed ? L.cin : L.cout, c1 = L.transposed ? L.cout : L.cin;
    int kf, kb;
    if (!L.transposed) { kf = 0; kb = L.mode == MODE_S1 ? 3 : 4; }
    else { kf = L.mode == MODE_S1 ? 1 : 2; kb = L.mode == MODE_S1 ? 5 : 6; }
    tab.e[2 * l] = {w, m->Gf[l], c0, c1, (kf == 0) ? 1 : 0, (kf == 1) ? 1 : 0};
    tab.e[2 * l + 1] = {w, m->Gb[l], c0, c1, (kb == 5 || kb == 6) ? 1 : 0, (kb == 3) ? 1 : 0};
  }
  tab.acc = m->bn_acc;
  tab.nacc = AVA_ACC_SLOTS * AVA_ACC_SLOT_LL;
  tab.keep0 = tab.keep1 = 0; tab.in_acc = nullptr;
  m->acc0_used = -1;
  mark(m, -1, st);
  if (x_stats != nullptr && nstats_out != nullptr && (reinterpret_cast<uintptr_t>(x_stats) & 15) == 0) {
    int64_t work = n / 4;
    int nstats = (int)((work + 256 * 8 - 1) / (256 * 8));
    if (nstats < 1) nstats = 1;
    if (nstats > 1024) nstats = 1024;
    int nnoise = ng.eps != nullptr ? (int)((ng.n + 255) / 256) : 0;
    if (nnoise > 64) nnoise = 64;
    hipStreamCaptureStatus cap = hipStreamCaptureStatusNone;
    const bool capturing = hipStreamIsCapturing(st, &cap) == hipSuccess && cap != hipStreamCaptureStatusNone;
    if (capturing) m->acc0_slot = -1;
    if (m->acc0_slot >= 0) {
      tab.in_acc = acc_slot(m, m->acc0_slot);
      tab.keep0 = m->acc0_slot * AVA_ACC_SLOT_LL; tab.keep1 = tab.keep0 + AVA_ACC_SLOT_LL;
      m->acc0_used = m->acc0_slot;
      m->acc0_slot = m->acc0_slot == 0 ? 28 : 0;
    } else {
      m->acc0_slot = capturing ? -1 : 0;
    }
    hipLaunchKernelGGL(pack_stats_kernel, dim3(nstats + 7 * 2 * NCONV + nnoise), dim3(256), 0, st, tab, x_stats, n, m->bn_part,
                       nstats, ng.eps, ng.n, ng.seed, ng.offset);
    AVA_CHECK_LAUNCH();
    *nstats_out = nstats;
    mark(m, CAT_PACK, st);
    return AVA_OK;
  }
  if (nstats_out != nullptr) *nstats_out = 0;
  if (ng.eps != nullptr) {
    TRY(ava_fill_normal(ng.eps, ng.n, ng.seed, ng.offset, reinterpret_cast<ava_stream_t>(st)));
    mark(m, CAT_LATENT_LOSS, st);
  }
  hipLaunchKernelGGL(pack_all_kernel, dim3(7, with_bwd ? 2 * NCONV : 2 * NCONV), dim3(256), 0, st, tab);
  AVA_CHECK_LAUNCH();
  {
    hipStreamCaptureStatus cap = hipStreamCaptureStatusNone;
    const bool capturing = hipStreamIsCapturing(st, &cap) == hipSuccess && cap != hipStreamCaptureStatusNone;
    m->acc0_slot = capturing ? -1 : 0;
  }
  mark(m, CAT_PACK, st);
  return AVA_OK;
}

static bool acc_pair_fwd(const ava_model* m, int j) {
  (void)m;
  return j >= 1 && j <= 13;
}
static bool acc_pair_bwd(const ava_model* m, int j) {
  (void)m;
  return j >= 0 && j <= 13;
}
static long long* acc_slot(ava_model* m, int slot) { return m->bn_acc + (size_t)slot * AVA_ACC_SLOT_LL; }
static BnFin fin_none() { BnFin f = {}; f.acc = nullptr; return f; }
static BnFin fin_fwd(ava_model* m, int j, int B) {
  const ConvLayer& L = kLayers[j];
  BnFin f = {};
  f.acc = acc_slot(m, j);
  f.gamma = PP(m, L.pg); f.beta = PP(m, L.pbeta);
  f.save = m->bn_save + (size_t)j * 4 * 32;
  f.running_mean = m->bn_running + j * 32;
  f.running_var = m->bn_running + (NCONV + j) * 32;
  f.num_batches = reinterpret_cast<long long*>(m->bn_batches + j);
  f.n = (double)B * m->lay[j].hi * m->lay[j].wi;
  f.C = L.cin; f.backward = 0; f.eval = 0;
  return f;
}
static BnFin fin_bwd(ava_model* m, int j, int B) {
  const ConvLayer& L = kLayers[j];
  BnFin f = {};
  f.acc = acc_slot(m, 14 + j);
  f.gamma = PP(m, L.pg);
  f.mean = bn_mean(m, j); f.invstd = bn_invstd(m, j);
  f.dgamma = GG(m, L.pg); f.dbeta = GG(m, L.pbeta);
  f.abc = m->bn_bwd + (size_t)j * 3 * 32;
  f.n = (double)B * m->lay[j].hi * m->lay[j].wi;
  f.C = L.cin; f.backward = 1; f.eval = m->last_train ? 0 : 1;
  return f;
}

static int finalize_fwd(ava_model* m, int l, int nparts, int64_t n, hipStream_t st) {
  const ConvLayer& L = kLayers[l];
  const int rc = ava_bn_finalize(m->bn_part, nparts, n, L.cin, PP(m, L.pg), PP(m, L.pbeta), m->bn_running + l * 32,
                                 m->bn_running + (NCONV + l) * 32, m->bn_batches + l, 1, bn_mean(m, l), bn_invstd(m, l),
                                 bn_scale(m, l), bn_shift(m, l), st);
  mark(m, CAT_BN, st);
  return rc;
}
static int finalize_bwd(ava_model* m, int l, int nparts, int64_t n, hipStream_t st) {
  const ConvLayer& L = kLayers[l];
  const int rc = ava_bn_finalize_bwd_ex(m->bn_part, nparts, n, L.cin, PP(m, L.pg), bn_mean(m, l), bn_invstd(m, l),
                                        GG(m, L.pg), GG(m, L.pbeta), bn_A(m, l), bn_B(m, l), bn_C(m, l),
                                        m->last_train ? 0 : 1, st);
  mark(m, CAT_BN, st);
  return rc;
}
static int bn_eval_all(ava_model* m, hipStream_t st) {
  const float* gamma[NCONV]; const float* beta[NCONV]; int C[NCONV];
  for (int l = 0; l < NCONV; ++l) { gamma[l] = PP(m, kLayers[l].pg); beta[l] = PP(m, kLayers[l].pbeta); C[l] = kLayers[l].cin; }
  const int rc = ava_bn_eval_all(gamma, beta, C, m->bn_running, m->bn_save, st);
  mark(m, CAT_BN, st);
  return rc;
}

static int gemm(ava_model* m, const float* A, int lda, const float* B, int ldb, const float* bias, float* C, int ldc,
                const float* mask, float* colsum, int M, int N, int K, int ak, int bk, int act, hipStream_t st) {
  struct Mk { ava_model* m; hipStream_t st; ~Mk() { mark(m, CAT_GEMM, st); } } _mk{m, st};
  return ava_gemm(A, lda, B, ldb, bias, C, ldc, mask, colsum, M, N, K, ak, bk, act, m->gemm_ws, m->gemm_ws_bytes, st);
}

static int gemm_defer2(ava_model* m, const float* A, int lda, const float* B, int ldb, const float* bias, float* C, int ldc,
                       int M, int N, int K, int ak, int bk, int act, hipStream_t st, int* slabs) {
  struct Mk { ava_model* m; hipStream_t st; ~Mk() { mark(m, CAT_GEMM, st); } } _mk{m, st};
  return ava_gemm_defer2(A, lda, B, ldb, bias, C, ldc, nullptr, nullptr, M, N, K, ak, bk, act, m->gemm_ws, m->gemm_ws_bytes, st, slabs);
}

struct AvaGemmProblem {
  const float* A; int lda; const float* B; int ldb; const float* bias; float* C; int ldc; const float* mask;
  float* colsum; int M, N, K; int act;
};
int ava_gemm_grouped(const AvaGemmProblem* p, int n, int a_kmajor, int b_kmajor, hipStream_t st);
static int gemm_group(ava_model* m, const AvaGemmProblem* p, int n, int ak, int bk, hipStream_t st) {
  const int rc = ava_gemm_grouped(p, n, ak, bk, st);
  mark(m, CAT_GEMM, st);
  return rc;
}

enum { FC1 = 28, FC2 = 30, FC31 = 32, FC32 = 34, FC33 = 36, FC41 = 38, FC42 = 40, FC43 = 42, FC5 = 44, FC6 = 46,
       FC7 = 48, FC8 = 50 };

static RecompArgs recomp_args(ava_model* m) {
  RecompArgs rc;
  rc.G1 = m->Gf[0]; rc.bias1 = PP(m, kLayers[0].pb); rc.pa1 = bn_scale(m, 0); rc.pb1 = bn_shift(m, 0);
  return rc;
}
extern "C" int ava_debug_materialize(ava_model* m, const float* x, int B, ava_stream_t s) {
  (void)s;
  if (m == nullptr || x == nullptr || B < 1 || B > m->maxB) return AVA_EINVAL;
  return AVA_OK;
}

static int encoder_forward(ava_model* m, const float* x, int B, int train, float* mu, float* u, float* logd_or_d,
                           int last_act, hipStream_t st, int pre_nparts = 0, bool stop_at_fc2 = false) {
  const int z = m->z;
  int nparts = pre_nparts;
  if (train) {
    if (nparts <= 0) {
      TRY(ava_bn_stats(x, (int64_t)B * m->H * m->W, 1, m->bn_part, &nparts, reinterpret_cast<ava_stream_t>(st)));
      mark(m, CAT_BN, st);
    }
    if (m->acc0_used < 0) TRY(finalize_fwd(m, 0, nparts, (int64_t)B * m->H * m->W, st));
  } else {
    TRY(bn_eval_all(m, st));
  }
  for (int l = 0; l < 7; ++l) {
    const ConvLayer& L = kLayers[l];
    const LayerDims& D = m->lay[l];
    const float* in = l == 0 ? x : m->X[l];
    float* out = l == 6 ? m->y7 : m->X[l + 1];
    float* nchw = l == 6 ? m->y7t : nullptr;
    ConvAcc acc;
    acc.fin = (train && acc_pair_fwd(m, l)) ? fin_fwd(m, l, B) : fin_none();
    if (train && l == 0 && m->acc0_used >= 0) { acc.fin = fin_fwd(m, 0, B); acc.fin.acc = acc_slot(m, m->acc0_used); }
    acc.acc_out = (train && l < 6 && acc_pair_fwd(m, l + 1)) ? acc_slot(m, l + 1) : nullptr;
    TRY(ava_conv3x3_ex(in, nullptr, bn_scale(m, l), bn_shift(m, l), nullptr, m->Gf[l], PP(m, L.pb), out, nchw,
                       nullptr, nullptr, nullptr, m->bn_part, B, D.hi, D.wi, L.cin, L.cout, L.mode, PRO_BN, EPI_FWD, 1,
                       0.f, m->act_bf16, &acc, reinterpret_cast<ava_stream_t>(st)));
    mark(m, CAT_CONV_FWD, st);
    if (train && l < 6 && acc.acc_out == nullptr)
      TRY(finalize_fwd(m, l + 1, ava_conv_grid(B, D.ho, D.wo, L.mode), (int64_t)B * D.ho * D.wo, st));
  }
  mark(m, CAT_LAYOUT, st);
  TRY(gemm(m, m->y7t, 0, PP(m, FC1), 0, PP(m, FC1 + 1), m->h1, 0, nullptr, nullptr, B, 1024, m->F, 1, 1, ACT_RELU, st));
  TRY(gemm(m, m->h1, 0, PP(m, FC2), 0, PP(m, FC2 + 1), m->h2, 0, nullptr, nullptr, B, 256, 1024, 1, 1, ACT_RELU, st));
  TRY(gemm(m, m->h2, 0, PP(m, FC31), 0, PP(m, FC31 + 1), m->h3, 0, nullptr, nullptr, B, 192, 256, 1, 1, ACT_RELU, st));
  if (stop_at_fc2) return AVA_OK;
  const AvaGemmProblem heads[3] = {
      {m->h3 + 0, 192, PP(m, FC41), 0, PP(m, FC41 + 1), mu, 0, nullptr, nullptr, B, z, 64, ACT_NONE},
      {m->h3 + 64, 192, PP(m, FC42), 0, PP(m, FC42 + 1), u, 0, nullptr, nullptr, B, z, 64, ACT_NONE},
      {m->h3 + 128, 192, PP(m, FC43), 0, PP(m, FC43 + 1), logd_or_d, 0, nullptr, nullptr, B, z, 64, last_act}};
  TRY(gemm_group(m, heads, 3, 1, 1, st));
  return AVA_OK;
}

static bool dd6_fused(const ava_model* m);
static bool acc_pair_bwd(const ava_model* m, int j);
static bool fold13_on(const ava_model* m) {
  return m->G != nullptr && acc_pair_bwd(m, 13) && m->lay[13].hi % 8 == 0;
}

static int decoder_forward(ava_model* m, const float* zin, const float* x_target, int B, int train, float* xrec,
                           hipStream_t st, bool from_fc7 = false, bool fold = false) {
  const int z = m->z;
  if (!from_fc7) {
    TRY(gemm(m, zin, 0, PP(m, FC5), 0, PP(m, FC5 + 1), m->h5, 0, nullptr, nullptr, B, 64, z, 1, 1, ACT_RELU, st));
    TRY(gemm(m, m->h5, 0, PP(m, FC6), 0, PP(m, FC6 + 1), m->h6, 0, nullptr, nullptr, B, 256, 64, 1, 1, ACT_RELU, st));
  }
  TRY(gemm(m, m->h6, 0, PP(m, FC7), 0, PP(m, FC7 + 1), m->h7, 0, nullptr, nullptr, B, 1024, 256, 1, 1, ACT_RELU, st));
  int slabs8 = 1;
  TRY(gemm_defer2(m, m->h7, 0, PP(m, FC8), 0, PP(m, FC8 + 1), m->f8, 0, B, m->F, 1024, 1, 1, ACT_RELU, st, &slabs8));
  int nparts = 0;
  long long* acc7 = (train && acc_pair_fwd(m, 7)) ? acc_slot(m, 7) : nullptr;
  if (slabs8 == 2) {
    const float* s0 = reinterpret_cast<const float*>(m->gemm_ws);
    TRY(ava_nchw_to_nhwc_stats_slabs(s0, s0 + (size_t)B * m->F, PP(m, FC8 + 1), 1, m->f8, m->X[7], m->bn_part, B, m->P8,
                                     m->act_bf16, acc7, &nparts, st));
  } else {
    TRY(ava_nchw_to_nhwc_stats(m->f8, m->X[7], m->bn_part, B, m->P8, m->act_bf16, acc7, &nparts, st));
  }
  mark(m, CAT_LAYOUT, st);
  if (train && acc7 == nullptr) TRY(finalize_fwd(m, 7, nparts, (int64_t)B * m->P8, st));
  for (int l = 7; l < NCONV; ++l) {
    const ConvLayer& L = kLayers[l];
    const LayerDims& D = m->lay[l];
    const bool last = l == NCONV - 1;
    float* out = last ? xrec : m->X[l + 1];
    ConvAcc acc;
    acc.fin = (train && acc_pair_fwd(m, l)) ? fin_fwd(m, l, B) : fin_none();
    acc.acc_out = (train && !last && acc_pair_fwd(m, l + 1)) ? acc_slot(m, l + 1) : nullptr;
    if (last && fold && train && x_target != nullptr && fold13_on(m)) {
      acc.fold.wg_partials = m->wg_part[l];
      acc.fold.acc_out = acc_slot(m, 14 + l);
      acc.fold.mean = bn_mean(m, l); acc.fold.invstd = bn_invstd(m, l);
      m->fold13 = 1;
      m->wg13_rows = ava_conv_grid(B, D.ho, D.wo, L.mode);
    }
    TRY(ava_conv3x3_ex(m->X[l], nullptr, bn_scale(m, l), bn_shift(m, l), nullptr, m->Gf[l], PP(m, L.pb), out,
                       last ? m->seed : nullptr, last ? x_target : nullptr, nullptr, nullptr, m->bn_part, B, D.hi, D.wi,
                       L.cin, L.cout, L.mode, PRO_BN, last ? EPI_SSE : EPI_FWD, 1, m->prec, m->act_bf16, &acc,
                       reinterpret_cast<ava_stream_t>(st)));
    mark(m, CAT_CONV_FWD, st);
    if (train && !last && acc.acc_out == nullptr)
      TRY(finalize_fwd(m, l + 1, ava_conv_grid(B, D.ho, D.wo, L.mode), (int64_t)B * D.ho * D.wo, st));
    if (last) m->sse_parts = ava_conv_grid(B, D.ho, D.wo, L.mode);
  }
  return AVA_OK;
}

static int forward_impl(ava_model* m, const float* x, int B, const float* eps_w, const float* eps_d, int bn_train,
                        float* loss_out, double* loss_accum, int* status_out, ava_stream_t s, NoiseGen ng) {
  if (m == nullptr || x == nullptr || eps_w == nullptr || eps_d == nullptr || B < 1 || B > m->maxB) return AVA_EINVAL;
  const ReserveScope rs(m);
  hipStream_t st = to_stream(s);
  const int z = m->z;
  int pre = 0;
  TRY(pack_weights(m, true, st, bn_train ? x : nullptr, (int64_t)B * m->H * m->W, &pre, ng));
  TRY(encoder_forward(m, x, B, bn_train, m->mu, m->u, m->logd, ACT_NONE, st, pre, true));
  mark(m, CAT_LAYOUT, st);
  FcMidFwdArgs fa;
  fa.h3_in = nullptr; fa.W3 = nullptr; fa.b3 = nullptr;
  fa.W41 = PP(m, FC41); fa.b41 = PP(m, FC41 + 1); fa.W42 = PP(m, FC42); fa.b42 = PP(m, FC42 + 1);
  fa.W43 = PP(m, FC43); fa.b43 = PP(m, FC43 + 1);
  fa.W5 = PP(m, FC5); fa.b5 = PP(m, FC5 + 1); fa.W6 = PP(m, FC6); fa.b6 = PP(m, FC6 + 1);
  fa.eps_w = eps_w; fa.eps_d = eps_d;
  fa.h3 = m->h3; fa.mu = m->mu; fa.u = m->u; fa.logd = m->logd; fa.d = m->d; fa.z = m->zs; fa.lat_sums = m->lat_sums;
  fa.h5 = m->h5; fa.h6 = m->h6; fa.status = status_out; fa.B = B; fa.zdim = z;
  TRY(ava_fc_mid_fwd(fa, st));
  m->eps_w_last = eps_w;
  m->eps_d_last = eps_d;
  mark(m, CAT_LATENT_LOSS, st);
  m->fold13 = 0;
  TRY(decoder_forward(m, m->zs, x, B, bn_train, m->xrec, st, true, true));
  TRY(ava_elbo_finalize_strided(m->lat_sums, B, m->bn_part, m->sse_parts, 2, z, m->prec, m->H * m->W,
                                loss_out != nullptr ? loss_out : m->loss_dev, loss_accum, st));
  mark(m, CAT_LATENT_LOSS, st);
  m->lastB = B;
  m->last_train = bn_train ? 1 : 0;
  m->status_last = status_out;
  m->bwd_scale = nullptr;
  return AVA_OK;
}

extern "C" int ava_forward(ava_model* m, const float* x, int B, const float* eps_w, const float* eps_d, int bn_train,
                           float* loss_out, double* loss_accum, int* status_out, ava_stream_t s) {
  return forward_impl(m, x, B, eps_w, eps_d, bn_train, loss_out, loss_accum, status_out, s, NoiseGen{nullptr, 0, 0, 0});
}

extern "C" int ava_forward_noise(ava_model* m, const float* x, int B, float* eps, uint64_t seed, uint64_t offset,
                                 int bn_train, float* loss_out, double* loss_accum, int* status_out, ava_stream_t s) {
  if (m == nullptr || eps == nullptr || B < 1) return AVA_EINVAL;
  const int64_t n = (int64_t)B * (m->z + 1);
  return forward_impl(m, x, B, eps, eps + B, bn_train, loss_out, loss_accum, status_out, s, NoiseGen{eps, n, seed, offset});
}

extern "C" int ava_encode(ava_model* m, const float* x, int B, int bn_train, float* mu, float* u, float* d,
                          ava_stream_t s) {
  if (m == nullptr || x == nullptr || mu == nullptr || u == nullptr || d == nullptr || B < 1 || B > m->maxB)
    return AVA_EINVAL;
  const ReserveScope rs(m);
  hipStream_t st = to_stream(s);
  m->lastB = 0;
  m->fold13 = 0;
  TRY(pack_weights(m, false, st));
  return encoder_forward(m, x, B, bn_train, mu, u, d, ACT_EXP, st);
}

extern "C" int ava_decode(ava_model* m, const float* z, int B, int bn_train, float* x_rec, ava_stream_t s) {
  if (m == nullptr || z == nullptr || x_rec == nullptr || B < 1 || B > m->maxB) return AVA_EINVAL;
  const ReserveScope rs(m);
  hipStream_t st = to_stream(s);
  m->lastB = 0;
  m->fold13 = 0;
  TRY(pack_weights(m, false, st));
  if (!bn_train) TRY(bn_eval_all(m, st));
  return decoder_forward(m, z, nullptr, B, bn_train, x_rec, st);
}

static int fused_grid(const ava_model* m, int l, int B) {
  const ConvLayer& L = kLayers[l];
  return ava_conv_fused_grid_for(B, m->lay[l].hi, m->lay[l].wi, L.cin, L.cout, L.mode);
}

static bool dd6_fused(const ava_model* m) {
  return fused_grid(m, 12, m->lastB > 0 ? m->lastB : 1) > 0 && m->lay[12].wi % 32 == 0 && m->lay[12].hi % 4 == 0;
}

int ava_conv3x3_wgrad_pair(const WgradCall& p, const WgradCall& q, int B, int act_bf16, ava_stream_t s);

static int conv_layer_backward(ava_model* m, int l, const float* x0, const float* gin, const float* gin2,
                               const float* ca, const float* cb, const float* cc, int pro, float* gout, int B,
                               hipStream_t st, WgradCall* defer = nullptr) {
  const ConvLayer& L = kLayers[l];
  const LayerDims& D = m->lay[l];
  const float* X = l == 0 ? x0 : m->X[l];
  const int fgrid = fused_grid(m, l, B);
  if (l == 13) {
    if (m->fold13 && dd6_fused(m)) return AVA_OK;
    if (m->fold13) {
      if (hipMemsetAsync(acc_slot(m, 14 + l), 0, (size_t)AVA_ACC_SLOT_LL * sizeof(long long), st) != hipSuccess) return AVA_ELAUNCH;
      m->fold13 = 0;
    }
    m->wg13_rows = fgrid;
  }
  if (fgrid > 0 && (gout != nullptr || l == 0)) {
    FusedArgs a = {};
    a.x = X; a.xa = bn_scale(m, l); a.xb = bn_shift(m, l);
    a.dy = gin; a.dy2 = gin2; a.da = ca; a.db = cb; a.dc = cc;
    a.Gb = m->Gb[l]; a.dx = gout; a.mean = bn_mean(m, l); a.invstd = bn_invstd(m, l);
    a.bn_partials = m->bn_part; a.wg_partials = m->wg_part[l];
    a.B = B; a.Hi = D.hi; a.Wi = D.wi; a.Ho = D.ho; a.Wo = D.wo;
    a.act_bf16 = m->act_bf16;
    const bool thin = L.cin == 1 || L.cout == 1;
    a.fin = ((!thin || l == 0) && pro == PRO_BWD && acc_pair_bwd(m, l + 1)) ? fin_bwd(m, l + 1, B) : fin_none();
    a.acc_out = ((!thin || l == 13 || l == 0) && acc_pair_bwd(m, l)) ? acc_slot(m, 14 + l) : nullptr;
    a.tiles_y = a.tiles_x = a.ntiles = 0;
    if (dd6_fused(m)) {
      if (l == 13) a.skip_dx = 1;
      if (l == 12) { a.dy = m->seed; a.rcd.G1 = m->Gb[13]; }
    }
    if (l == 0 && pro == PRO_BWD) a.rc = recomp_args(m);
    TRY(ava_conv3x3_bwd_fused_launch(a, L.cin, L.cout, L.mode, pro, st));
    mark(m, CAT_CONV_BWD_DATA, st);
    if (a.acc_out != nullptr) return AVA_OK;
    return finalize_bwd(m, l, fgrid, (int64_t)B * D.hi * D.wi, st);
  }
  const int bmode = L.mode == MODE_S1 ? MODE_S1 : (L.mode == MODE_DOWN ? MODE_UP : MODE_DOWN);
  ConvAcc acc;
  acc.fin = (pro == PRO_BWD && acc_pair_bwd(m, l + 1)) ? fin_bwd(m, l + 1, B) : fin_none();
  acc.acc_out = acc_pair_bwd(m, l) ? acc_slot(m, 14 + l) : nullptr;
  TRY(ava_conv3x3_ex(gin, gin2, ca, cb, cc, m->Gb[l], nullptr, gout, nullptr, X, bn_mean(m, l), bn_invstd(m, l),
                     m->bn_part, B, D.ho, D.wo, L.cout, L.cin, bmode, pro, EPI_BWD, 0, 0.f, m->act_bf16, &acc,
                     reinterpret_cast<ava_stream_t>(st)));
  mark(m, CAT_CONV_BWD_DATA, st);
  if (acc.acc_out == nullptr) TRY(finalize_bwd(m, l, ava_conv_grid(B, D.hi, D.wi, bmode), (int64_t)B * D.hi * D.wi, st));
  if (defer != nullptr) {
    *defer = WgradCall{X, bn_scale(m, l), bn_shift(m, l), gin, gin2, ca, cb, cc, m->wg_part[l], D.hi, D.wi, L.cin, L.cout, L.mode, pro};
    return AVA_OK;
  }
  TRY(ava_conv3x3_wgrad_ex(X, bn_scale(m, l), bn_shift(m, l), gin, gin2, ca, cb, cc, m->wg_part[l], B, D.hi, D.wi, L.cin,
                           L.cout, L.mode, pro, m->act_bf16, st));
  mark(m, CAT_CONV_WGRAD, st);
  return AVA_OK;
}

static int reduce_wgrads(ava_model* m, int l0, int l1, int B, hipStream_t st) {
  WgradReduceTable tab;
  int blocks = 0, n = 0;
  for (int l = l0; l < l1; ++l, ++n) {
    const ConvLayer& L = kLayers[l];
    tab.e[n].partials = m->wg_part[l];
    tab.e[n].dw = GG(m, L.pw);
    tab.e[n].dbias = GG(m, L.pb);
    const int fg = l == 13 && m->wg13_rows > 0 ? m->wg13_rows : fused_grid(m, l, B);
    tab.e[n].nparts = fg > 0 ? fg : ava_conv_wgrad_rows_ex(B, m->lay[l].hi, m->lay[l].wi, L.cin, L.cout, L.mode, l == 13 || l == 6 ? PRO_ID : PRO_BWD, m->act_bf16);
    tab.e[n].cin = L.cin; tab.e[n].cout = L.cout;
    tab.e[n].kind = !L.transposed ? 0 : (L.mode == MODE_S1 ? 1 : 2);
    tab.e[n].block0 = blocks;
    blocks += ceil_div(9 * L.cin * L.cout + L.cout, 32);
  }
  tab.n = n;
  tab.fin0 = (l0 == 0 && acc_pair_bwd(m, 0)) ? fin_bwd(m, 0, B) : fin_none();
  TRY(ava_conv_wgrad_reduce_all(tab, blocks, st));
  mark(m, CAT_CONV_WGRAD, st);
  return AVA_OK;
}

#define AVA_BACKWARD_PARTS 4
extern "C" int ava_backward_num_parts(void) { return AVA_BACKWARD_PARTS; }
extern "C" int ava_grad_bucket(ava_model* m, int bucket, int64_t* offset, int64_t* count) {
  if (m == nullptr || offset == nullptr || count == nullptr || bucket < 0 || bucket >= AVA_BACKWARD_PARTS) return AVA_EINVAL;
  const int64_t fc1 = m->tab[28].off, fc1b = m->tab[29].off, fc8 = m->tab[50].off;
  if (bucket == 0) { *offset = fc8; *count = m->arena - fc8; }
  else if (bucket == 1) { *offset = fc1; *count = fc1b - fc1; }
  else if (bucket == 2) { *offset = fc1b; *count = fc8 - fc1b; }
  else { *offset = 0; *count = fc1; }
  return AVA_OK;
}

static int backward_part0(ava_model* m, const float* x, int B, hipStream_t st, bool whole);
static int backward_part1(ava_model* m, const float* x, int B, hipStream_t st);
static int backward_part1b(ava_model* m, const float* x, int B, hipStream_t st);
static int backward_part2(ava_model* m, const float* x, int B, hipStream_t st, bool whole);

extern "C" int ava_set_backward_scale(ava_model* m, const float* loss_scale) {
  if (m == nullptr) return AVA_EINVAL;
  m->bwd_scale = loss_scale;
  return AVA_OK;
}

extern "C" int ava_backward(ava_model* m, const float* x, int B, ava_stream_t s) {
  if (m == nullptr || x == nullptr || B != m->lastB || m->G == nullptr) return AVA_EINVAL;
  const ReserveScope rs(m);
  TRY(backward_part0(m, x, B, to_stream(s), true));
  TRY(backward_part1(m, x, B, to_stream(s)));
  TRY(backward_part1b(m, x, B, to_stream(s)));
  return backward_part2(m, x, B, to_stream(s), true);
}
extern "C" int ava_backward_part(ava_model* m, const float* x, int B, int part, ava_stream_t s) {
  if (m == nullptr || x == nullptr || B != m->lastB || m->G == nullptr || part < 0 || part >= AVA_BACKWARD_PARTS)
    return AVA_EINVAL;
  const ReserveScope rs(m);
  if (part == 0) return backward_part0(m, x, B, to_stream(s), false);
  if (part == 1) return backward_part1(m, x, B, to_stream(s));
  if (part == 2) return backward_part1b(m, x, B, to_stream(s));
  return backward_part2(m, x, B, to_stream(s), false);
}

static size_t grad_half(const ava_model* m, int B) { return (size_t)B * m->H * m->W * 4; }

static int backward_part0(ava_model* m, const float* x, int B, hipStream_t st, bool whole) {
  float* gcur = m->gA;
  float* gnext = m->gB;
  mark(m, -1, st);
  if (m->bwd_scale != nullptr) {
    const bool folded = m->fold13 && dd6_fused(m);
    TRY(ava_scale_backward_roots(m->seed, (int64_t)B * m->H * m->W, folded ? m->wg_part[13] : nullptr,
                                 folded ? (int64_t)m->wg13_rows * 73 : 0, folded ? acc_slot(m, 14 + 13) : nullptr, m->bwd_scale, st));
    mark(m, CAT_LAYOUT, st);
  }
  TRY(conv_layer_backward(m, 13, x, m->seed, nullptr, nullptr, nullptr, nullptr, PRO_ID, gcur, B, st));
  const bool pair = fused_grid(m, 8, B) == 0 && fused_grid(m, 7, B) == 0;
  WgradCall wc[2];
  for (int l = 12; l >= 7; --l) {
    float* gout = (pair && l == 7) ? gnext + grad_half(m, B) : gnext;
    TRY(conv_layer_backward(m, l, x, gcur, m->X[l + 1], bn_A(m, l + 1), bn_B(m, l + 1), bn_C(m, l + 1), PRO_BWD, gout,
                            B, st, pair && l <= 8 ? &wc[8 - l] : nullptr));
    gnext = gcur; gcur = gout;
  }
  if (pair) {
    TRY(ava_conv3x3_wgrad_pair(wc[0], wc[1], B, m->act_bf16, reinterpret_cast<ava_stream_t>(st)));
    mark(m, CAT_CONV_WGRAD, st);
  }
  const BnFin fin8 = acc_pair_bwd(m, 7) ? fin_bwd(m, 7, B) : fin_none();
  TRY(ava_bn_bwd_apply_to_nchw(gcur, m->f8, bn_A(m, 7), bn_B(m, 7), bn_C(m, 7), m->dF8, B, m->P8, m->act_bf16, &fin8, st));
  mark(m, CAT_LAYOUT, st);
  if (!whole) TRY(reduce_wgrads(m, 7, NCONV, B, st));
  TRY(gemm(m, m->dF8, 0, m->h7, 0, nullptr, GG(m, FC8), 0, nullptr, GG(m, FC8 + 1), m->F, 1024, B, 0, 0, ACT_NONE, st));
  return AVA_OK;
}

static int backward_part1(ava_model* m, const float* x, int B, hipStream_t st) {
  const int z = m->z;
  mark(m, -1, st);
  TRY(gemm(m, m->dF8, 0, PP(m, FC8), 0, nullptr, m->dh7, 0, m->h7, nullptr, B, 1024, m->F, 1, 0, ACT_NONE, st));
  TRY(gemm(m, m->dh7, 0, PP(m, FC7), 0, nullptr, m->dh6, 0, m->h6, nullptr, B, 256, 1024, 1, 0, ACT_NONE, st));
  FcMidBwdArgs ba;
  ba.dh6 = m->dh6; ba.W6 = PP(m, FC6); ba.W5 = PP(m, FC5); ba.W41 = PP(m, FC41); ba.W42 = PP(m, FC42); ba.W43 = PP(m, FC43);
  ba.W3 = PP(m, FC31); ba.h5 = m->h5; ba.h3 = m->h3; ba.h2 = m->h2;
  ba.z = m->zs; ba.u = m->u; ba.d = m->d; ba.eps_w = m->eps_w_last; ba.eps_d = m->eps_d_last; ba.scale = m->bwd_scale;
  ba.dh5 = m->dh5; ba.dz = m->dz; ba.dmu = m->dmu; ba.du = m->du; ba.dlogd = m->dlogd; ba.dh3 = m->dh3; ba.dh2 = m->dh2;
  ba.B = B; ba.zdim = z;
  TRY(ava_fc_mid_bwd(ba, st));
  mark(m, CAT_LATENT_LOSS, st);
  TRY(gemm(m, m->dh3, 0, PP(m, FC31), 0, nullptr, m->dh2, 0, m->h2, nullptr, B, 256, 192, 1, 0, ACT_NONE, st));
  TRY(gemm(m, m->dh2, 0, PP(m, FC2), 0, nullptr, m->dh1, 0, m->h1, nullptr, B, 1024, 256, 1, 0, ACT_NONE, st));
  return gemm(m, m->dh1, 0, m->y7t, 0, nullptr, GG(m, FC1), 0, nullptr, GG(m, FC1 + 1), 1024, m->F, B, 0, 0, ACT_NONE, st);
}

static int backward_part1b(ava_model* m, const float* x, int B, hipStream_t st) {
  const int z = m->z;
  (void)x;
  mark(m, -1, st);
  m->dy7_slabs = 1;
  {
    struct Mk { ava_model* m; hipStream_t st; ~Mk() { mark(m, CAT_GEMM, st); } } _mk{m, st};
    TRY(ava_gemm_defer2(m->dh1, 0, PP(m, FC1), 0, nullptr, m->dy7, 0, nullptr, nullptr, B, m->F, 1024, 1, 0, ACT_NONE,
                        m->dy7_ws, m->dy7_ws_bytes, st, &m->dy7_slabs));
  }
  const AvaGemmProblem dws[8] = {
      {m->dh7, 0, m->h6, 0, nullptr, GG(m, FC7), 0, nullptr, GG(m, FC7 + 1), 1024, 256, B, ACT_NONE},
      {m->dh6, 0, m->h5, 0, nullptr, GG(m, FC6), 0, nullptr, GG(m, FC6 + 1), 256, 64, B, ACT_NONE},
      {m->dh5, 0, m->zs, 0, nullptr, GG(m, FC5), 0, nullptr, GG(m, FC5 + 1), 64, z, B, ACT_NONE},
      {m->dmu, 0, m->h3 + 0, 192, nullptr, GG(m, FC41), 0, nullptr, GG(m, FC41 + 1), z, 64, B, ACT_NONE},
      {m->du, 0, m->h3 + 64, 192, nullptr, GG(m, FC42), 0, nullptr, GG(m, FC42 + 1), z, 64, B, ACT_NONE},
      {m->dlogd, 0, m->h3 + 128, 192, nullptr, GG(m, FC43), 0, nullptr, GG(m, FC43 + 1), z, 64, B, ACT_NONE},
      {m->dh3, 0, m->h2, 0, nullptr, GG(m, FC31), 0, nullptr, GG(m, FC31 + 1), 192, 256, B, ACT_NONE},
      {m->dh2, 0, m->h1, 0, nullptr, GG(m, FC2), 0, nullptr, GG(m, FC2 + 1), 256, 1024, B, ACT_NONE}};
  return gemm_group(m, dws, 8, 0, 0, st);
}

static int backward_part2(ava_model* m, const float* x, int B, hipStream_t st, bool whole) {
  float* gcur = m->gA;
  float* gnext = m->gB;
  mark(m, -1, st);
  if (m->dy7_slabs == 2) {
    const float* s0 = reinterpret_cast<const float*>(m->dy7_ws);
    TRY(ava_relu_mask_to_nhwc(s0, s0 + (size_t)B * m->F, m->y7, gcur, B, m->P8, st));
  } else {
    TRY(ava_relu_mask_to_nhwc(m->dy7, nullptr, m->y7, gcur, B, m->P8, st));
  }
  mark(m, CAT_LAYOUT, st);
  const bool pair = fused_grid(m, 6, B) == 0 && fused_grid(m, 5, B) == 0;
  WgradCall wc[2];
  TRY(conv_layer_backward(m, 6, x, gcur, nullptr, nullptr, nullptr, nullptr, PRO_ID, gnext, B, st, pair ? &wc[0] : nullptr));
  { float* t = gcur; gcur = gnext; gnext = t; }
  bool upper = false;
  for (int l = 5; l >= 0; --l) {
    float* gout = l == 0 ? nullptr : ((pair && l == 5) ? gnext + grad_half(m, B) : gnext);
    TRY(conv_layer_backward(m, l, x, gcur, m->X[l + 1], bn_A(m, l + 1), bn_B(m, l + 1), bn_C(m, l + 1), PRO_BWD, gout, B, st,
                            pair && l == 5 ? &wc[1] : nullptr));
    if (pair && l == 5) {
      TRY(ava_conv3x3_wgrad_pair(wc[0], wc[1], B, m->act_bf16, reinterpret_cast<ava_stream_t>(st)));
      mark(m, CAT_CONV_WGRAD, st);
    }
    float* freed = upper ? gcur - grad_half(m, B) : gcur;
    gcur = gout; gnext = freed;
    upper = pair && l == 5;
  }
  m->bwd_scale = nullptr;
  return reduce_wgrads(m, whole ? 0 : 0, whole ? NCONV : 7, B, st);
}

extern "C" int ava_adam_step_range(ava_model* m, int64_t offset, int64_t count, double lr, double beta1, double beta2,
                                   double eps, int step, ava_stream_t s) {
  if (m == nullptr || m->G == nullptr || m->M == nullptr || m->V == nullptr || offset < 0 || count <= 0 ||
      offset + count > m->arena || offset % 4 != 0 || count % 4 != 0)
    return AVA_EINVAL;
  const ReserveScope rs(m);
  mark(m, -1, to_stream(s));
  const int rc = ava_adam_flat_guarded(m->P + offset, m->G + offset, m->M + offset, m->V + offset, count, lr, beta1, beta2,
                                       eps, step, m->status_last, to_stream(s));
  mark(m, CAT_ADAM, to_stream(s));
  return rc;
}

extern "C" int ava_adam_step(ava_model* m, double lr, double beta1, double beta2, double eps, int step,
                             ava_stream_t s) {
  if (m == nullptr || m->G == nullptr || m->M == nullptr || m->V == nullptr) return AVA_EINVAL;
  const ReserveScope rs(m);
  mark(m, -1, to_stream(s));
  const int rc = ava_adam_flat_guarded(m->P, m->G, m->M, m->V, m->arena, lr, beta1, beta2, eps, step, m->status_last,
                                       to_stream(s));
  mark(m, CAT_ADAM, to_stream(s));
  return rc;
}
```

include/ava_hip.h:

```cpp
#ifndef AVA_HIP_H
#define AVA_HIP_H

#include <stddef.h>
#include <stdint.h>

#ifdef __cplusplus
extern "C" {
#endif

#define AVA_OK 0
#define AVA_EINVAL (-1)
#define AVA_ELAUNCH (-2)
#define AVA_EWORKSPACE (-3)

typedef void* ava_stream_t;
typedef struct ava_model ava_model;

int ava_version(void);
int64_t ava_arena_floats(int z_dim);
int64_t ava_param_offset(int z_dim, int index, int64_t* numel);
size_t ava_workspace_bytes(int z_dim, int max_batch);

int ava_model_create(ava_model** out, int z_dim, int max_batch, float model_precision,
                     float* params, float* grads, float* exp_avg, float* exp_avg_sq,
                     float* bn_running, int64_t* bn_batches, void* workspace, size_t workspace_bytes);
void ava_model_destroy(ava_model* m);
int64_t ava_arena_floats_hw(int z_dim, int H, int W);
int64_t ava_param_offset_hw(int z_dim, int H, int W, int index, int64_t* numel);
size_t ava_workspace_bytes_hw(int z_dim, int H, int W, int max_batch);
int ava_model_create_hw(ava_model** out, int z_dim, int H, int W, int max_batch, float model_precision,
                        float* params, float* grads, float* exp_avg, float* exp_avg_sq,
                        float* bn_running, int64_t* bn_batches, void* workspace, size_t workspace_bytes);
int ava_model_create_ex(ava_model** out, int z_dim, int H, int W, int act_dtype, int max_batch, float model_precision,
                        float* params, float* grads, float* exp_avg, float* exp_avg_sq,
                        float* bn_running, int64_t* bn_batches, void* workspace, size_t workspace_bytes);

int ava_forward(ava_model* m, const float* x, int B, const float* eps_w, const float* eps_d,
                int bn_train, float* loss_out, double* loss_accum, int* status_out, ava_stream_t s);
int ava_forward_noise(ava_model* m, const float* x, int B, float* eps, uint64_t seed, uint64_t offset,
                      int bn_train, float* loss_out, double* loss_accum, int* status_out, ava_stream_t s);
int ava_backward(ava_model* m, const float* x, int B, ava_stream_t s);
int ava_set_backward_scale(ava_model* m, const float* loss_scale);
int ava_backward_num_parts(void);
int ava_backward_part(ava_model* m, const float* x, int B, int part, ava_stream_t s);
int ava_grad_bucket(ava_model* m, int bucket, int64_t* offset, int64_t* count);
int ava_set_cu_reserve(int cus);
int ava_get_cu_reserve(void);
int ava_model_set_cu_reserve(ava_model* m, int cus);
int ava_model_get_cu_reserve(const ava_model* m);
int ava_occupy_cus(int workgroups, int lds_bytes, float usec, ava_stream_t s);
int ava_adam_step(ava_model* m, double lr, double beta1, double beta2, double eps, int step, ava_stream_t s);
int ava_adam_step_range(ava_model* m, int64_t offset, int64_t count, double lr, double beta1, double beta2, double eps,
                        int step, ava_stream_t s);
int ava_encode(ava_model* m, const float* x, int B, int bn_train, float* mu, float* u, float* d, ava_stream_t s);
int ava_decode(ava_model* m, const float* z, int B, int bn_train, float* x_rec, ava_stream_t s);
const float* ava_last_z(ava_model* m);
const float* ava_last_xrec(ava_model* m);
const float* ava_debug_buffer(ava_model* m, const char* name, int64_t* floats);
int ava_debug_materialize(ava_model* m, const float* x, int B, ava_stream_t s);

#define AVA_PROFILE_CATEGORIES 9
int ava_profile_enable(ava_model* m, int on);
int ava_profile_read(ava_model* m, float* ms, int* launches);

int ava_fill_normal(float* out, int64_t n, uint64_t seed, uint64_t offset, ava_stream_t s);

int ava_pack_conv_weight(const float* w, float* g, int c_first, int c_second, int kind, ava_stream_t s);

int ava_conv_grid(int B, int Ho, int Wo, int mode);
int ava_conv3x3(const float* in, const float* in2, const float* pa, const float* pb, const float* pc,
                const float* G, const float* bias, float* out, float* out2,
                const float* epi_x, const float* epi_mean, const float* epi_invstd, float* partials,
                int B, int Hi, int Wi, int Cin, int Cout, int mode, int pro, int epi, int relu, float prec,
                ava_stream_t s);
int ava_conv3x3_wgrad(const float* x, const float* xa, const float* xb,
                      const float* dy, const float* dy2, const float* da, const float* db_, const float* dc,
                      float* partials, int B, int Hi, int Wi, int Cin, int Cout, int mode, int dy_pro,
                      ava_stream_t s);
int ava_conv_wgrad_grid(int B, int Ho, int Wo, int mode);
int ava_conv_wgrad_rows(int B, int Hi, int Wi, int Cin, int Cout, int mode, int dy_pro);
int ava_conv_fused_grid(int B, int Hi, int Wi, int Cin, int Cout, int mode);
int ava_conv3x3_bwd_fused(const float* x, const float* xa, const float* xb,
                          const float* dy, const float* dy2, const float* da, const float* db_, const float* dc,
                          const float* Gb, float* dx, const float* mean, const float* invstd,
                          float* bn_partials, float* wg_partials,
                          int B, int Hi, int Wi, int Cin, int Cout, int mode, int dy_pro, ava_stream_t s);
int ava_conv_wgrad_reduce(const float* partials, int nparts, float* dw, float* dbias,
                          int Cin, int Cout, int kind, ava_stream_t s);

int ava_bn_stats(const float* x, int64_t n, int C, float* partials, int* nparts, ava_stream_t s);
int ava_bn_finalize(const float* partials, int nparts, int64_t n, int C, const float* gamma, const float* beta,
                    float* running_mean, float* running_var, int64_t* num_batches, int train,
                    float* mean, float* invstd, float* scale, float* shift, ava_stream_t s);
int ava_bn_finalize_bwd(const float* partials, int nparts, int64_t n, int C, const float* gamma,
                        const float* mean, const float* invstd, float* dgamma, float* dbeta,
                        float* A, float* Bc, float* Cc, ava_stream_t s);

size_t ava_gemm_workspace_bytes(int M, int N, int K);
int ava_gemm(const float* A, int lda, const float* B, int ldb, const float* bias, float* C, int ldc,
             const float* mask, float* colsum, int M, int N, int K, int a_kmajor, int b_kmajor, int act,
             void* ws, size_t ws_bytes, ava_stream_t s);

int ava_latent_fwd(const float* mu, const float* u, const float* logd, const float* eps_w, const float* eps_d,
                   float* d, float* z, float* sums, int* status, int B, int zdim, ava_stream_t s);
int ava_latent_bwd(const float* z, const float* dz_dec, const float* u, const float* d, const float* eps_w,
                   const float* eps_d, float* dmu, float* du, float* dlogd, int B, int zdim, ava_stream_t s);
int ava_elbo_finalize(const float* latent_sums, int B, const float* sse_partials, int nparts,
                      int zdim, float prec, float* loss_out, ava_stream_t s);
int ava_adam_flat(float* p, const float* g, float* m, float* v, int64_t n, double lr, double beta1, double beta2,
                  double eps, int step, ava_stream_t s);

int ava_cast_to_f32(const void* src, int src_dtype, int64_t n, float* dst, ava_stream_t s);
int ava_host_gather_rows(void* dst, const void* src, const int64_t* idx, int64_t first, int64_t n, size_t row_bytes,
                         int threads);

size_t ava_mmd2_workspace_bytes(int n1, int n2);
int ava_mmd2(const double* latent, int z, const int64_t* i1, int n1, const int64_t* i2, int n2, double sigma,
             double* out4, void* ws, size_t ws_bytes, ava_stream_t s);
int ava_mmd2_linear(const double* latent, int z, const int64_t* i1, const int64_t* i2, int m, double sigma,
                    double* out, void* ws, size_t ws_bytes, ava_stream_t s);
int ava_pair_sqdist(const double* latent, int z, const int64_t* a, const int64_t* b, int n, double* out,
                    ava_stream_t s);

size_t ava_spec_workspace_bytes(int n, int max_samples, int nperseg, int noverlap, int F, int T, int normalize);
int ava_get_spec_batch(const void* audio, int audio_dtype, const int64_t* file_off, const int64_t* file_len,
                       const int32_t* file_idx, const double* t1, const double* t2, const double* target_times,
                       int n, int max_samples, double fs, int nperseg, int noverlap, const double* window,
                       double scale, const double* target_freqs, int F, int T, double spec_min, double spec_max,
                       double fill_value, int remove_dc, int normalize, int q_lo, double q_gamma, float* out,
                       float* out_max, void* ws, size_t ws_bytes, ava_stream_t s);

size_t ava_amp_workspace_bytes(int64_t frames);
int ava_amp_trace(const void* audio, int audio_dtype, const int64_t* file_off, const int64_t* file_len,
                  const int64_t* frame_off, int files, int64_t frames, int nperseg, int noverlap, const double* window,
                  double scale, int k0, int k1, double spec_min, double spec_max, int softmax, double temperature,
                  const double* gauss_w, int radius, int trace_f64, void* trace, double* spec, void* ws,
                  size_t ws_bytes, ava_stream_t s);
int ava_amp_decide(const void* trace, int trace_f64, const int64_t* frame_off, int files, int64_t frames, double th1,
                   double th2, double th3, uint64_t* count, int64_t* maxima, int64_t* left, int64_t* right,
                   int64_t capacity, ava_stream_t s);

size_t ava_tpl_workspace_bytes(int64_t lags);
int ava_tpl_tile_lags(void);
int ava_tpl_spec(const void* audio, int audio_dtype, const int64_t* file_off, const int64_t* file_len,
                 const int64_t* frame_off, int files, int64_t frames, int nperseg, int noverlap, const double* window,
                 double scale, int k0, int k1, double spec_min, double spec_max, double* spec, double* frame_sum,
                 ava_stream_t s);
int ava_tpl_xcorr(const double* spec, const double* frame_sum, int F, int64_t frames, const int64_t* frame_off,
                  const int64_t* lag_off, const int64_t* tile_off, int files, int64_t lags, int64_t tiles,
                  const double* tmpl, int template_F, int L, double* trace, void* ws, size_t ws_bytes, ava_stream_t s);

size_t ava_warp_cache_bytes(int files, double template_dur, double fs, int nperseg, int noverlap, double fmin,
                            double fmax);
int ava_warp_cache_layout(int files, double template_dur, double fs, int nperseg, int noverlap, double fmin, double fmax,
                          int64_t out[6]);
size_t ava_warp_cache_workspace_bytes(int files, double template_dur, double fs, int nperseg, int noverlap);
int ava_warp_cache_build(const void* audio, int audio_dtype, const int64_t* file_off, const int64_t* file_len, int files,
                         double template_dur, double fs, int nperseg, int noverlap, const double* window, double scale,
                         double fmin, double fmax, int remove_dc, void* cache, size_t cache_bytes, void* ws,
                         size_t ws_bytes, ava_stream_t s);
size_t ava_warp_windows_workspace_bytes(int n, int F, int T, int normalize);
int ava_warp_windows(const void* cache, size_t cache_bytes, int files, double template_dur, double fs, int nperseg,
                     int noverlap, double fmin, double fmax, const int32_t* file_idx, const double* target_times, int n,
                     const double* target_freqs, int F, int T, double spec_min, double spec_max, double fill_value,
                     int normalize, int q_lo, double q_gamma, float* out, void* ws, size_t ws_bytes, ava_stream_t s);
int ava_warp_band_spec(const void* audio, int audio_dtype, const int64_t* file_off, const int64_t* file_len,
                       const int64_t* frame_off, int files, int64_t frames, int nperseg, int noverlap,
                       const double* window, double scale, int k0, int k1, double spec_min, double divisor, double* spec,
                       double* frame_sum, ava_stream_t s);

size_t ava_nn_workspace_bytes(int nq, int nr, int d, int metric);
int ava_nn_argmin(const void* queries, int q_dtype, int nq, const void* refs, int r_dtype, int nr, int d, int metric,
                  int64_t* out_idx, double* out_dist, void* ws, size_t ws_bytes, ava_stream_t s);
int ava_nn_merge(int64_t* best_idx, double* best_dist, const int64_t* idx, const double* dist, int nq, int64_t offset,
                 int metric, ava_stream_t s);

int ava_pj_knn(const void* x, int dtype, int n, int d, int k, int q0, int nq, int64_t* out_idx, double* out_dist,
               ava_stream_t s);
int ava_pj_smooth(const double* dist, const int64_t* idx, int n, int k, double local_connectivity, double* mean_all,
                  double* sigma, double* rho, double* w, ava_stream_t s);
int ava_pj_layout(double* y, double* y_tmp, const int64_t* indptr, const int* col, const double* eps,
                  const double* epn, double* next_s, double* next_n, int n, int64_t nnz, int e0, int e1, int n_epochs,
                  double learning_rate, double a, double b, double gamma, uint64_t salt, int* flag, ava_stream_t s);
size_t ava_pj_gram_workspace_bytes(int n, int d);
int ava_pj_gram(const void* x, int dtype, int n, int d, double* gram, void* ws, size_t ws_bytes, ava_stream_t s);
int ava_pj_project(const void* x, int dtype, int n, int d, const double* V, const double* muv, int nc, double* out,
                   ava_stream_t s);

#ifdef __cplusplus
}
#endif
#endif
```

Before: 179,200 spectrograms/s.

## Pre-split fc1/fc8 activations into bf16 limb planes reused across GEMMs

Adds a limb-split kernel that converts the fp32 activations and gradients feeding fc1 and fc8 (y7t, h7, dF8, dh1) into three bf16 limb planes once, in both k-major and transposed layouts. The limb GEMM kernel gains loaders that read these pre-split planes directly, so repeated fp32-to-limb conversion and transposition inside the GEMM stager is skipped for forward, data-gradient and weight-gradient products. The bias gradient column sum is folded into the split pass. In exchange it adds extra split launches, plane buffers in the arena and more kernel template variants, and only pays off if the planes are reused enough to cover the split cost.

After: 177,200 spectrograms/s. -1.1%, worse.

```diff
diff --git a/autoencoded-vocal-analysis_amd/_lib.py b/autoencoded-vocal-analysis_amd/_lib.py
--- a/autoencoded-vocal-analysis_amd/_lib.py
+++ b/autoencoded-vocal-analysis_amd/_lib.py
@@ -82,6 +82,10 @@
     "ava_bn_finalize_bwd": (_i, [_p, _i, _i64, _i, _p, _p, _p, _p, _p, _p, _p, _p, _p]),
     "ava_gemm_workspace_bytes": (_sz, [_i, _i, _i]),
     "ava_gemm": (_i, [_p, _i, _p, _i, _p, _p, _i, _p, _p, _i, _i, _i, _i, _i, _i, _p, _sz, _p]),
+    "ava_limb_planes_bytes": (_sz, [_i, _i]),
+    "ava_limb_split": (_i, [_p, _i, _i, _i, _p, _p, _p, _p]),
+    "ava_gemm_planes_used": (_i, [_i, _i, _i, _i, _i]),
+    "ava_gemm_planes": (_i, [_p, _i, _p, _p, _i, _p, _p, _p, _i, _p, _p, _i, _i, _i, _i, _i, _i, _p, _sz, _p]),
     "ava_latent_fwd": (_i, [_p] * 9 + [_i, _i, _p]),
     "ava_latent_bwd": (_i, [_p] * 9 + [_i, _i, _p]),
     "ava_elbo_finalize": (_i, [_p, _i, _p, _i, _i, _f, _p, _p]),
diff --git a/autoencoded-vocal-analysis_amd/csrc/gemm.h b/autoencoded-vocal-analysis_amd/csrc/gemm.h
--- a/autoencoded-vocal-analysis_amd/csrc/gemm.h
+++ b/autoencoded-vocal-analysis_amd/csrc/gemm.h
@@ -16,6 +16,19 @@
   int splits;
   int act;
   int vec_a, vec_b;
+  const uint16_t* Ap;
+  const uint16_t* Bp;
+  int ldap, ldbp;
+  size_t psa, psb;
+};
+
+static inline int limb_plane_ld(int K) { return (K + 31) / 32 * 32; }
+static inline size_t limb_plane_elems(int rows, int K) { return (size_t)3 * rows * limb_plane_ld(K); }
+
+struct GemmOperand {
+  const float* f32;
+  int ld;
+  const uint16_t* planes;
 };
 
 #ifdef __HIPCC__
@@ -29,3 +42,9 @@
 bool ava_gemm_limb_ok(const GemmArgs& g, int a_kmajor, int b_kmajor);
 void ava_gemm_limb_plan(int M, int N, int K, int a_kmajor, int* bn, int* splits, int* klen);
 int ava_gemm_limb_launch(const GemmArgs& g, int a_kmajor, int b_kmajor, int bn, hipStream_t st);
+bool ava_gemm_planes_ok(int M, int N, int K, int a_kmajor, int b_kmajor);
+int ava_limb_split_launch(const float* X, int ldx, int R, int C, uint16_t* planes_k, uint16_t* planes_t, float* colsum,
+                          hipStream_t st);
+int ava_gemm_operands(const GemmOperand& A, const GemmOperand& B, const float* bias, float* C, int ldc, const float* mask,
+                      float* colsum, int M, int N, int K, int a_kmajor, int b_kmajor, int act, void* ws, size_t ws_bytes,
+                      ava_stream_t s, int* slabs);
diff --git a/autoencoded-vocal-analysis_amd/csrc/gemm.hip b/autoencoded-vocal-analysis_amd/csrc/gemm.hip
--- a/autoencoded-vocal-analysis_amd/csrc/gemm.hip
+++ b/autoencoded-vocal-analysis_amd/csrc/gemm.hip
@@ -426,7 +426,40 @@
 
 static int gemm_impl(const float* A, int lda, const float* B, int ldb, const float* bias, float* C, int ldc,
                      const float* mask, float* colsum, int M, int N, int K, int a_kmajor, int b_kmajor, int act,
-                     void* ws, size_t ws_bytes, ava_stream_t s, int* deferred_slabs);
+                     void* ws, size_t ws_bytes, ava_stream_t s, int* deferred_slabs, const uint16_t* Ap = nullptr,
+                     const uint16_t* Bp = nullptr);
+
+int ava_gemm_operands(const GemmOperand& A, const GemmOperand& B, const float* bias, float* C, int ldc, const float* mask,
+                      float* colsum, int M, int N, int K, int a_kmajor, int b_kmajor, int act, void* ws, size_t ws_bytes,
+                      ava_stream_t s, int* slabs) {
+  if (slabs != nullptr) *slabs = 1;
+  if (M <= 0 || N <= 0 || K <= 0) return AVA_EINVAL;
+  const bool both = !a_kmajor && !b_kmajor;
+  const size_t pmax = (size_t)(M > N ? M : N) * limb_plane_ld(K);
+  const bool use = ava_gemm_planes_ok(M, N, K, a_kmajor, b_kmajor) && A.planes != nullptr && pmax < ((size_t)1 << 31) &&
+                   (!both || (B.planes != nullptr && colsum == nullptr)) &&
+                   ((reinterpret_cast<uintptr_t>(A.planes) | (both ? reinterpret_cast<uintptr_t>(B.planes) : 0)) & 15) == 0;
+  return gemm_impl(A.f32, A.ld, B.f32, B.ld, bias, C, ldc, mask, colsum, M, N, K, a_kmajor, b_kmajor, act, ws, ws_bytes, s,
+                   slabs, use ? A.planes : nullptr, use && both ? B.planes : nullptr);
+}
+
+extern "C" size_t ava_limb_planes_bytes(int rows, int K) {
+  return rows > 0 && K > 0 ? limb_plane_elems(rows, K) * sizeof(uint16_t) : 0;
+}
+extern "C" int ava_limb_split(const float* X, int ldx, int R, int C, void* planes_k, void* planes_t, float* colsum,
+                              ava_stream_t s) {
+  return ava_limb_split_launch(X, ldx, R, C, reinterpret_cast<uint16_t*>(planes_k), reinterpret_cast<uint16_t*>(planes_t),
+                               colsum, to_stream(s));
+}
+extern "C" int ava_gemm_planes_used(int M, int N, int K, int a_kmajor, int b_kmajor) {
+  return ava_gemm_planes_ok(M, N, K, a_kmajor, b_kmajor) ? 1 : 0;
+}
+extern "C" int ava_gemm_planes(const float* A, int lda, const void* a_planes, const float* B, int ldb, const void* b_planes,
+                               const float* bias, float* C, int ldc, const float* mask, float* colsum, int M, int N, int K,
+                               int a_kmajor, int b_kmajor, int act, void* ws, size_t ws_bytes, ava_stream_t s) {
+  const GemmOperand a{A, lda, reinterpret_cast<const uint16_t*>(a_planes)}, b{B, ldb, reinterpret_cast<const uint16_t*>(b_planes)};
+  return ava_gemm_operands(a, b, bias, C, ldc, mask, colsum, M, N, K, a_kmajor, b_kmajor, act, ws, ws_bytes, s, nullptr);
+}
 
 extern "C" int ava_gemm(const float* A, int lda, const float* B, int ldb, const float* bias, float* C, int ldc,
                         const float* mask, float* colsum, int M, int N, int K, int a_kmajor, int b_kmajor, int act,
@@ -443,8 +476,9 @@
 
 static int gemm_impl(const float* A, int lda, const float* B, int ldb, const float* bias, float* C, int ldc,
                      const float* mask, float* colsum, int M, int N, int K, int a_kmajor, int b_kmajor, int act,
-                     void* ws, size_t ws_bytes, ava_stream_t s, int* deferred_slabs) {
-  if (A == nullptr || B == nullptr || C == nullptr || M <= 0 || N <= 0 || K <= 0) return AVA_EINVAL;
+                     void* ws, size_t ws_bytes, ava_stream_t s, int* deferred_slabs, const uint16_t* Ap, const uint16_t* Bp) {
+  if ((A == nullptr && Ap == nullptr) || (B == nullptr && Bp == nullptr) || C == nullptr || M <= 0 || N <= 0 || K <= 0)
+    return AVA_EINVAL;
   int bm, splits, klen;
   plan(M, N, K, &bm, &splits, &klen);
   if (splits > 1 && (ws == nullptr || ws_bytes < ava_gemm_workspace_bytes(M, N, K))) return AVA_EWORKSPACE;
@@ -458,7 +492,13 @@
   g.klen = klen; g.splits = splits; g.act = act;
   g.vec_a = (g.lda % 4 == 0) && ((reinterpret_cast<uintptr_t>(A) & 15) == 0) && (a_kmajor ? K % 4 == 0 && K >= 4 : M % 4 == 0 && M >= 4);
   g.vec_b = (g.ldb % 4 == 0) && ((reinterpret_cast<uintptr_t>(B) & 15) == 0) && (b_kmajor ? K % 4 == 0 && K >= 4 : N % 4 == 0 && N >= 4);
-  const bool vec = g.vec_a && g.vec_b;
+  g.Ap = Ap; g.Bp = Bp;
+  g.ldap = g.ldbp = limb_plane_ld(K);
+  g.psa = (size_t)M * g.ldap; g.psb = (size_t)N * g.ldbp;
+  const int vec_a32 = g.vec_a, vec_b32 = g.vec_b;
+  if (Ap != nullptr) g.vec_a = 1;
+  if (Bp != nullptr) g.vec_b = 1;
+  const bool vec = vec_a32 && vec_b32;
   hipStream_t st = to_stream(s);
   if (ava_gemm_limb_ok(g, a_kmajor, b_kmajor)) {
     int lbn;
@@ -483,6 +523,8 @@
     }
     return AVA_OK;
   }
+  if ((Ap != nullptr && A == nullptr) || (Bp != nullptr && B == nullptr)) return AVA_EINVAL;
+  g.Ap = g.Bp = nullptr; g.vec_a = vec_a32; g.vec_b = vec_b32;
   if (skinny_ok(g, a_kmajor, b_kmajor)) {
     g.C = C;
     const dim3 sgrid(ceil_div(N, 16), ceil_div(M, 16));
diff --git a/autoencoded-vocal-analysis_amd/csrc/gemm_limb.hip b/autoencoded-vocal-analysis_amd/csrc/gemm_limb.hip
--- a/autoencoded-vocal-analysis_amd/csrc/gemm_limb.hip
+++ b/autoencoded-vocal-analysis_amd/csrc/gemm_limb.hip
@@ -165,12 +165,47 @@
   }
 };
 
-template <int BT, int T, int RING, bool KMAJ>
+template <int BT, int T, int LIMB_RING>
+struct LimbLoaderP {
+  static constexpr int UNITS = BT * 4, NU = (UNITS + T - 1) / T;
+  u32x4 r[LIMB_RING][NU][3];
+  unsigned off[NU];
+  __device__ __forceinline__ void init(int t0, int extent, int ld) {
+#pragma unroll
+    for (int i = 0; i < NU; ++i) {
+      const int u = threadIdx.x + T * i, row = u >> 2, oct = u & 3;
+      off[i] = (unsigned)min(t0 + row, extent - 1) * (unsigned)ld + oct * 8;
+    }
+  }
+  template <int SLOT>
+  __device__ __forceinline__ void load(const uint16_t* __restrict__ base, size_t ps, int ld, int k0, int ) {
+    const uint16_t* b = base + min(k0, ld - LBK);
+#pragma unroll
+    for (int i = 0; i < NU; ++i)
+#pragma unroll
+      for (int l = 0; l < 3; ++l) r[SLOT][i][l] = *reinterpret_cast<const u32x4*>(b + l * ps + off[i]);
+  }
+  template <int SLOT, bool COLSUM>
+  __device__ __forceinline__ void store(unsigned char* __restrict__ S) {
+#pragma unroll
+    for (int i = 0; i < NU; ++i) {
+      const int u = threadIdx.x + T * i, row = u >> 2, oct = u & 3;
+      if (UNITS % T != 0 && u >= UNITS) continue;
+      unsigned char* d = S + row * 64 + chunk_of<false>(row & 15, oct) * 16;
+#pragma unroll
+      for (int l = 0; l < 3; ++l) *reinterpret_cast<u32x4*>(d + l * BT * 64) = r[SLOT][i][l];
+    }
+  }
+};
+
+template <int BT, int T, int RING, bool KMAJ, bool PLANES>
 struct LimbLoader;
 template <int BT, int T, int RING>
-struct LimbLoader<BT, T, RING, true> : LimbLoaderK<BT, T, RING> {};
+struct LimbLoader<BT, T, RING, true, false> : LimbLoaderK<BT, T, RING> {};
 template <int BT, int T, int RING>
-struct LimbLoader<BT, T, RING, false> : LimbLoaderN<BT, T, RING> {};
+struct LimbLoader<BT, T, RING, false, false> : LimbLoaderN<BT, T, RING> {};
+template <int BT, int T, int RING, bool KMAJ>
+struct LimbLoader<BT, T, RING, KMAJ, true> : LimbLoaderP<BT, T, RING> {};
 
 template <int J, int R, class F>
 __device__ __forceinline__ void limb_for_stage(F&& f) {
@@ -180,7 +215,7 @@
 
 struct LimbItem { int m0, n0, split, kbeg, kend, bx; };
 
-template <int BN, bool A_KMAJ, bool B_KMAJ, int RING, int MINW>
+template <int BN, bool A_KMAJ, bool B_KMAJ, int RING, int MINW, bool A_PL = false, bool B_PL = false>
 __global__ __launch_bounds__(512, MINW) void gemm_limb_kernel(const GemmArgs g, const int tiles_m, const int tiles_n,
                                                               const int nitems) {
   constexpr int NSW = 4;
@@ -212,32 +247,54 @@
 
   if (stager) {
     __builtin_amdgcn_s_setprio(3);
-    LimbLoader<BM, T, RING, A_KMAJ> la;
-    LimbLoader<BN, T, RING, B_KMAJ> lb;
+    LimbLoader<BM, T, A_PL ? 1 : RING, A_KMAJ, A_PL> la;
+    LimbLoader<BN, T, RING, B_KMAJ, B_PL> lb;
     int S = 0;
     for (int i = it; i < it_end; i += it_step) { const LimbItem q = decode(i); S += (q.kend - q.kbeg + LBK - 1) / LBK; }
     int l_it = it, s_it = it;
     LimbItem li = decode(l_it), si = li;
     int l_k = li.kbeg, s_k = si.kbeg;
+    int a_it = it;
+    LimbItem ai = li;
+    int a_k = ai.kbeg;
+    auto a_load = [&]() __attribute__((always_inline)) {
+      if constexpr (A_PL) {
+        if (a_k == ai.kbeg) la.init(ai.m0, g.M, g.ldap);
+        la.template load<0>(g.Ap, g.psa, g.ldap, a_k, ai.kend);
+        a_k += LBK;
+        if (a_k >= ai.kend) {
+          a_it += it_step;
+          if (a_it < it_end) { ai = decode(a_it); a_k = ai.kbeg; }
+        }
+      }
+    };
     auto load_step = [&](auto slot) __attribute__((always_inline)) {
       constexpr int SLOT = decltype(slot)::value;
-      if (l_k == li.kbeg) { la.init(li.m0, g.M, g.lda); lb.init(li.n0, g.N, g.ldb); }
-      la.template load<SLOT>(g.A, g.lda, l_k, li.kend, g.K);
-      lb.template load<SLOT>(g.B, g.ldb, l_k, li.kend, g.K);
+      if (l_k == li.kbeg) {
+        if constexpr (!A_PL) la.init(li.m0, g.M, g.lda);
+        lb.init(li.n0, g.N, B_PL ? g.ldbp : g.ldb);
+      }
+      if constexpr (!A_PL) la.template load<SLOT>(g.A, g.lda, l_k, li.kend, g.K);
+      if constexpr (B_PL) lb.template load<SLOT>(g.Bp, g.psb, g.ldbp, l_k, li.kend);
+      else lb.template load<SLOT>(g.B, g.ldb, l_k, li.kend, g.K);
       l_k += LBK;
       if (l_k >= li.kend) {
         l_it += it_step;
         if (l_it < it_end) { li = decode(l_it); l_k = li.kbeg; }
       }
     };
-    auto store_step = [&](auto slot, int buf) __attribute__((always_inline)) {
+    auto store_step = [&](auto slot, int buf, auto always) __attribute__((always_inline)) {
       constexpr int SLOT = decltype(slot)::value;
       unsigned char* S_ = smem + buf * BUF;
-      la.template store<SLOT, !A_KMAJ>(S_);
+      la.template store<A_PL ? 0 : SLOT, !A_KMAJ && !A_PL>(S_);
+      if constexpr (A_PL) {
+        if constexpr (decltype(always)::value) a_load();
+        else if (a_it < it_end) a_load();
+      }
       lb.template store<SLOT, false>(S_ + A_BYTES);
       s_k += LBK;
       if (s_k >= si.kend) {
-        if constexpr (!A_KMAJ) {
+        if constexpr (!A_KMAJ && !A_PL) {
           if (g.colsum != nullptr && si.bx == 0) {
             const bool fin = g.splits == 1;
 #pragma unroll
@@ -267,14 +324,15 @@
       }
     };
     limb_for_stage<0, RING - 1>([&](auto J) __attribute__((always_inline)) { if (decltype(J)::value < S) load_step(J); });
-    store_step(std::integral_constant<int, 0>{}, 0);
+    if constexpr (A_PL) a_load();
+    store_step(std::integral_constant<int, 0>{}, 0, std::false_type{});
     __syncthreads();
     int s0 = 0;
     for (; s0 + 2 * RING - 2 < S; s0 += RING)
       limb_for_stage<0, RING>([&](auto J) __attribute__((always_inline)) {
         constexpr int j = decltype(J)::value;
         load_step(std::integral_constant<int, (j + RING - 1) % RING>{});
-        store_step(std::integral_constant<int, (j + 1) % RING>{}, (s0 + j + 1) & 1);
+        store_step(std::integral_constant<int, (j + 1) % RING>{}, (s0 + j + 1) & 1, std::true_type{});
         __syncthreads();
       });
     for (; s0 < S; s0 += RING)
@@ -282,7 +340,7 @@
         constexpr int j = decltype(J)::value;
         if (s0 + j < S) {
           if (s0 + j + RING - 1 < S) load_step(std::integral_constant<int, (j + RING - 1) % RING>{});
-          if (s0 + j + 1 < S) store_step(std::integral_constant<int, (j + 1) % RING>{}, (s0 + j + 1) & 1);
+          if (s0 + j + 1 < S) store_step(std::integral_constant<int, (j + 1) % RING>{}, (s0 + j + 1) & 1, std::false_type{});
           __syncthreads();
         }
       });
@@ -291,8 +349,9 @@
 
   const int wave = wave8 - NSW, wm = wave >> 1, wn = wave & 1;
   const int fr = lane & 15, kg = lane >> 4;
-  const int a_lane = (wm * WM) * 64 + pos16<!A_KMAJ>(fr) * 64 + chunk_of<!A_KMAJ>(fr, kg) * 16;
-  const int b_lane = A_BYTES + (wn * WN) * 64 + pos16<!B_KMAJ>(fr) * 64 + chunk_of<!B_KMAJ>(fr, kg) * 16;
+  constexpr bool A_PERM = !A_KMAJ && !A_PL, B_PERM = !B_KMAJ && !B_PL;
+  const int a_lane = (wm * WM) * 64 + pos16<A_PERM>(fr) * 64 + chunk_of<A_PERM>(fr, kg) * 16;
+  const int b_lane = A_BYTES + (wn * WN) * 64 + pos16<B_PERM>(fr) * 64 + chunk_of<B_PERM>(fr, kg) * 16;
   f32x4 acc[TM][TN];
   __syncthreads();
   int s = 0;
@@ -425,7 +484,15 @@
   }
   const int resident = ava_scale_grid((bn == 64 ? 2 : 1) * cus);
   int grid = nitems < resident ? nitems : resident;
-  if (bn == 64 && a_kmajor) {
+  const bool apl = g.Ap != nullptr, bpl = g.Bp != nullptr;
+  if (apl || bpl) {
+    if (bn == 64 && a_kmajor && apl && !bpl) {
+      if (b_kmajor) hipLaunchKernelGGL((gemm_limb_kernel<64, true, true, 3, 4, true, false>), dim3(grid), dim3(512), 0, st, g, tm, tn, nitems);
+      else hipLaunchKernelGGL((gemm_limb_kernel<64, true, false, 3, 4, true, false>), dim3(grid), dim3(512), 0, st, g, tm, tn, nitems);
+    } else if (bn == 128 && !a_kmajor && !b_kmajor && apl && bpl && g.colsum == nullptr) {
+      hipLaunchKernelGGL((gemm_limb_kernel<128, false, false, 3, 2, true, true>), dim3(grid), dim3(512), 0, st, g, tm, tn, nitems);
+    } else return AVA_EINVAL;
+  } else if (bn == 64 && a_kmajor) {
     if (b_kmajor) hipLaunchKernelGGL((gemm_limb_kernel<64, true, true, 3, 4>), dim3(grid), dim3(512), 0, st, g, tm, tn, nitems);
     else hipLaunchKernelGGL((gemm_limb_kernel<64, true, false, 3, 4>), dim3(grid), dim3(512), 0, st, g, tm, tn, nitems);
   } else if (bn == 128 && !a_kmajor) {
@@ -436,3 +503,135 @@
   AVA_CHECK_LAUNCH();
   return AVA_OK;
 }
+
+__device__ __forceinline__ void limb_split8(const float* v, u32x4& p0, u32x4& p1, u32x4& p2) {
+#pragma unroll
+  for (int j = 0; j < 4; ++j) {
+    uint32_t x, y, z;
+    limb_split2(v[2 * j], v[2 * j + 1], x, y, z);
+    p0[j] = x; p1[j] = y; p2[j] = z;
+  }
+}
+
+struct LimbSplitArgs {
+  const float* X;
+  uint16_t* pk;
+  uint16_t* pt;
+  float* colsum;
+  int R, C, ldx, ldk, ldt;
+  int nk, nt;
+  int vec;
+};
+
+__global__ __launch_bounds__(256) void limb_split_kernel(const LimbSplitArgs a) {
+  __shared__ float tile[32][65];
+  const int t = threadIdx.x, b = blockIdx.x;
+  if (b < a.nk) {
+    const int upr = a.ldk >> 3;
+    const size_t total = (size_t)a.R * upr, ps = (size_t)a.R * a.ldk;
+    for (size_t u = (size_t)b * 256 + t; u < total; u += (size_t)a.nk * 256) {
+      const int row = (int)(u / upr), c0 = (int)(u - (size_t)row * upr) * 8;
+      const float* src = a.X + (size_t)row * a.ldx + c0;
+      float v[8];
+      if (a.vec && c0 + 8 <= a.C) {
+        const float4 lo = *reinterpret_cast<const float4*>(src), hi = *reinterpret_cast<const float4*>(src + 4);
+        v[0] = lo.x; v[1] = lo.y; v[2] = lo.z; v[3] = lo.w; v[4] = hi.x; v[5] = hi.y; v[6] = hi.z; v[7] = hi.w;
+      } else {
+#pragma unroll
+        for (int j = 0; j < 8; ++j) v[j] = c0 + j < a.C ? src[j] : 0.f;
+      }
+      u32x4 p0, p1, p2;
+      limb_split8(v, p0, p1, p2);
+      uint16_t* d = a.pk + (size_t)row * a.ldk + c0;
+      *reinterpret_cast<u32x4*>(d) = p0;
+      *reinterpret_cast<u32x4*>(d + ps) = p1;
+      *reinterpret_cast<u32x4*>(d + 2 * ps) = p2;
+    }
+    return;
+  }
+  if (b < a.nk + a.nt) {
+    const int tr = a.ldt >> 5, tb = b - a.nk;
+    const int cb = tb / tr, r0 = (tb - cb * tr) * 32, c0 = cb * 64;
+#pragma unroll
+    for (int i = 0; i < 2; ++i) {
+      const int r = (t >> 4) + 16 * i, c = 4 * (t & 15), gr = r0 + r, gc = c0 + c;
+      float4 x = make_float4(0.f, 0.f, 0.f, 0.f);
+      if (gr < a.R) {
+        const float* src = a.X + (size_t)gr * a.ldx + gc;
+        if (a.vec && gc + 4 <= a.C) x = *reinterpret_cast<const float4*>(src);
+        else {
+          if (gc + 0 < a.C) x.x = src[0];
+          if (gc + 1 < a.C) x.y = src[1];
+          if (gc + 2 < a.C) x.z = src[2];
+          if (gc + 3 < a.C) x.w = src[3];
+        }
+      }
+      tile[r][c + 0] = x.x; tile[r][c + 1] = x.y; tile[r][c + 2] = x.z; tile[r][c + 3] = x.w;
+    }
+    __syncthreads();
+    const int c = t >> 2, oct = t & 3;
+    if (c0 + c < a.C) {
+      float v[8];
+#pragma unroll
+      for (int j = 0; j < 8; ++j) v[j] = tile[oct * 8 + j][c];
+      u32x4 p0, p1, p2;
+      limb_split8(v, p0, p1, p2);
+      const size_t ps = (size_t)a.C * a.ldt;
+      uint16_t* d = a.pt + (size_t)(c0 + c) * a.ldt + r0 + oct * 8;
+      *reinterpret_cast<u32x4*>(d) = p0;
+      *reinterpret_cast<u32x4*>(d + ps) = p1;
+      *reinterpret_cast<u32x4*>(d + 2 * ps) = p2;
+    }
+    return;
+  }
+  float (*part)[32] = reinterpret_cast<float (*)[32]>(&tile[0][0]);
+  const int kq = t >> 5, c = t & 31, gc = (b - a.nk - a.nt) * 32 + c;
+  const bool in = gc < a.C;
+  const float* col = a.X + (in ? gc : 0);
+  float cs = 0.f;
+  for (int k0 = 0; k0 < a.R; k0 += LBK) {
+    float v[4];
+#pragma unroll
+    for (int j = 0; j < 4; ++j) {
+      const int gk = k0 + 4 * kq + j;
+      const float x = col[(size_t)min(gk, a.R - 1) * a.ldx];
+      v[j] = (in && gk < a.R) ? x : 0.f;
+    }
+    cs += (v[0] + v[1]) + (v[2] + v[3]);
+  }
+  part[kq][c] = cs;
+  __syncthreads();
+  if (kq == 0 && in)
+    a.colsum[gc] = ((part[0][c] + part[1][c]) + (part[2][c] + part[3][c])) + ((part[4][c] + part[5][c]) + (part[6][c] + part[7][c]));
+}
+
+int ava_limb_split_launch(const float* X, int ldx, int R, int C, uint16_t* planes_k, uint16_t* planes_t, float* colsum,
+                          hipStream_t st) {
+  if (X == nullptr || R < 1 || C < 1) return AVA_EINVAL;
+  if (((reinterpret_cast<uintptr_t>(planes_k) | reinterpret_cast<uintptr_t>(planes_t)) & 15) != 0) return AVA_EINVAL;
+  LimbSplitArgs a;
+  a.X = X; a.pk = planes_k; a.pt = planes_t; a.colsum = colsum;
+  a.R = R; a.C = C; a.ldx = ldx > 0 ? ldx : C;
+  a.ldk = limb_plane_ld(C); a.ldt = limb_plane_ld(R);
+  a.vec = (a.ldx % 4 == 0) && ((reinterpret_cast<uintptr_t>(X) & 15) == 0);
+  a.nk = a.nt = 0;
+  if (planes_k != nullptr) {
+    const size_t units = (size_t)R * (a.ldk / 8);
+    a.nk = (int)((units + 255) / 256 < 4096 ? (units + 255) / 256 : 4096);
+  }
+  if (planes_t != nullptr) a.nt = (a.ldt / 32) * ceil_div(C, 64);
+  const int nc = colsum != nullptr ? ceil_div(C, 32) : 0;
+  if (a.nk + a.nt + nc == 0) return AVA_OK;
+  hipLaunchKernelGGL(limb_split_kernel, dim3(a.nk + a.nt + nc), dim3(256), 0, st, a);
+  AVA_CHECK_LAUNCH();
+  return AVA_OK;
+}
+
+bool ava_gemm_planes_ok(int M, int N, int K, int a_kmajor, int b_kmajor) {
+  if (!limb_shape(M, N, K) || N % 4 != 0) return false;
+  if (a_kmajor) return K % 8 == 0;
+  if (b_kmajor || M % 4 != 0) return false;
+  int bn, splits, klen;
+  ava_gemm_limb_plan(M, N, K, 0, &bn, &splits, &klen);
+  return splits == 1;
+}
diff --git a/autoencoded-vocal-analysis_amd/csrc/model.hip b/autoencoded-vocal-analysis_amd/csrc/model.hip
--- a/autoencoded-vocal-analysis_amd/csrc/model.hip
+++ b/autoencoded-vocal-analysis_amd/csrc/model.hip
@@ -24,6 +24,13 @@
 int ava_gemm_defer2(const float* A, int lda, const float* B, int ldb, const float* bias, float* C, int ldc,
                     const float* mask, float* colsum, int M, int N, int K, int a_kmajor, int b_kmajor, int act,
                     void* ws, size_t ws_bytes, ava_stream_t s, int* slabs);
+struct GemmOperand { const float* f32; int ld; const uint16_t* planes; };
+int ava_gemm_operands(const GemmOperand& A, const GemmOperand& B, const float* bias, float* C, int ldc, const float* mask,
+                      float* colsum, int M, int N, int K, int a_kmajor, int b_kmajor, int act, void* ws, size_t ws_bytes,
+                      ava_stream_t s, int* slabs);
+bool ava_gemm_planes_ok(int M, int N, int K, int a_kmajor, int b_kmajor);
+int ava_limb_split_launch(const float* X, int ldx, int R, int C, uint16_t* planes_k, uint16_t* planes_t, float* colsum,
+                          hipStream_t st);
 int ava_bn_bwd_apply_to_nchw(const float* g, const float* f8, const float* A, const float* Bc, const float* Cc,
                              float* out, int B, int P, int act_bf16, const BnFin* fin, hipStream_t st);
 int ava_bn_finalize_bwd_ex(const float* partials, int nparts, int64_t n, int C, const float* gamma, const float* mean,
@@ -163,6 +170,7 @@
   int cu_reserve;
   float* wg_part[NCONV];
   float *dF8, *dh7, *dh6, *dh5, *dz, *dmu, *du, *dlogd, *dh3, *dh2, *dh1, *dy7;
+  uint16_t *y7t_k, *y7t_t, *h7_k, *h7_t, *dF8_k, *dF8_t, *dh1_k, *dh1_t;
   float* gemm_ws;
   size_t gemm_ws_bytes;
   float* loss_dev;
@@ -268,6 +276,11 @@
   m->dF8 = c.take(B * F); m->dh7 = c.take(B * 1024); m->dh6 = c.take(B * 256); m->dh5 = c.take(B * 64);
   m->dz = c.take(B * z); m->dmu = c.take(B * z); m->du = c.take(B * z); m->dlogd = c.take(B * z);
   m->dh3 = c.take(B * 192); m->dh2 = c.take(B * 256); m->dh1 = c.take(B * 1024); m->dy7 = c.take(B * F);
+  {
+    auto planes = [&](size_t rows, size_t k) { return reinterpret_cast<uint16_t*>(c.take((3 * rows * ((k + 31) / 32 * 32) + 1) / 2)); };
+    m->y7t_k = planes(B, F); m->y7t_t = planes(F, B); m->h7_k = planes(B, 1024); m->h7_t = planes(1024, B);
+    m->dF8_k = planes(B, F); m->dF8_t = planes(F, B); m->dh1_k = planes(B, 1024); m->dh1_t = planes(1024, B);
+  }
   m->gemm_ws_bytes = max_gemm_ws(z, (int)B, m->F);
   m->gemm_ws = c.take(m->gemm_ws_bytes / sizeof(float) + 64);
   m->dy7_ws_bytes = max_dy7_ws((int)B, m->F);
@@ -685,6 +698,23 @@
   return ava_gemm_defer2(A, lda, B, ldb, bias, C, ldc, nullptr, nullptr, M, N, K, ak, bk, act, m->gemm_ws, m->gemm_ws_bytes, st, slabs);
 }
 
+static int gemm_pl(ava_model* m, const GemmOperand& A, const GemmOperand& B, const float* bias, float* C, const float* mask,
+                   float* colsum, int M, int N, int K, int ak, int bk, int act, hipStream_t st, int* slabs = nullptr,
+                   void* ws = nullptr, size_t ws_bytes = 0) {
+  struct Mk { ava_model* m; hipStream_t st; ~Mk() { mark(m, CAT_GEMM, st); } } _mk{m, st};
+  return ava_gemm_operands(A, B, bias, C, 0, mask, colsum, M, N, K, ak, bk, act, ws != nullptr ? ws : m->gemm_ws,
+                           ws != nullptr ? ws_bytes : m->gemm_ws_bytes, st, slabs);
+}
+static int split_act(ava_model* m, const float* X, int B, int C, uint16_t* pk, bool fwd_ok, uint16_t* pt, bool dw_ok,
+                     float* colsum, hipStream_t st) {
+  if (!fwd_ok) pk = nullptr;
+  if (!dw_ok) { pt = nullptr; colsum = nullptr; }
+  if (pk == nullptr && pt == nullptr) return AVA_OK;
+  const int rc = ava_limb_split_launch(X, 0, B, C, pk, pt, colsum, st);
+  mark(m, CAT_LAYOUT, st);
+  return rc;
+}
+
 struct AvaGemmProblem {
   const float* A; int lda; const float* B; int ldb; const float* bias; float* C; int ldc; const float* mask;
   float* colsum; int M, N, K; int act;
@@ -741,7 +771,10 @@
       TRY(finalize_fwd(m, l + 1, ava_conv_grid(B, D.ho, D.wo, L.mode), (int64_t)B * D.ho * D.wo, st));
   }
   mark(m, CAT_LAYOUT, st);
-  TRY(gemm(m, m->y7t, 0, PP(m, FC1), 0, PP(m, FC1 + 1), m->h1, 0, nullptr, nullptr, B, 1024, m->F, 1, 1, ACT_RELU, st));
+  const bool y_k = ava_gemm_planes_ok(B, 1024, m->F, 1, 1), y_t = stop_at_fc2 && ava_gemm_planes_ok(1024, m->F, B, 0, 0);
+  TRY(split_act(m, m->y7t, B, m->F, m->y7t_k, y_k, m->y7t_t, y_t, nullptr, st));
+  TRY(gemm_pl(m, {m->y7t, 0, y_k ? m->y7t_k : nullptr}, {PP(m, FC1), 0, nullptr}, PP(m, FC1 + 1), m->h1, nullptr, nullptr, B,
+              1024, m->F, 1, 1, ACT_RELU, st));
   TRY(gemm(m, m->h1, 0, PP(m, FC2), 0, PP(m, FC2 + 1), m->h2, 0, nullptr, nullptr, B, 256, 1024, 1, 1, ACT_RELU, st));
   TRY(gemm(m, m->h2, 0, PP(m, FC31), 0, PP(m, FC31 + 1), m->h3, 0, nullptr, nullptr, B, 192, 256, 1, 1, ACT_RELU, st));
   if (stop_at_fc2) return AVA_OK;
@@ -768,7 +801,10 @@
   }
   TRY(gemm(m, m->h6, 0, PP(m, FC7), 0, PP(m, FC7 + 1), m->h7, 0, nullptr, nullptr, B, 1024, 256, 1, 1, ACT_RELU, st));
   int slabs8 = 1;
-  TRY(gemm_defer2(m, m->h7, 0, PP(m, FC8), 0, PP(m, FC8 + 1), m->f8, 0, B, m->F, 1024, 1, 1, ACT_RELU, st, &slabs8));
+  const bool h_k = ava_gemm_planes_ok(B, m->F, 1024, 1, 1), h_t = fold && ava_gemm_planes_ok(m->F, 1024, B, 0, 0);
+  TRY(split_act(m, m->h7, B, 1024, m->h7_k, h_k, m->h7_t, h_t, nullptr, st));
+  TRY(gemm_pl(m, {m->h7, 0, h_k ? m->h7_k : nullptr}, {PP(m, FC8), 0, nullptr}, PP(m, FC8 + 1), m->f8, nullptr, nullptr, B,
+              m->F, 1024, 1, 1, ACT_RELU, st, &slabs8));
   int nparts = 0;
   long long* acc7 = (train && acc_pair_fwd(m, 7)) ? acc_slot(m, 7) : nullptr;
   if (slabs8 == 2) {
@@ -1035,14 +1071,18 @@
   TRY(ava_bn_bwd_apply_to_nchw(gcur, m->f8, bn_A(m, 7), bn_B(m, 7), bn_C(m, 7), m->dF8, B, m->P8, m->act_bf16, &fin8, st));
   mark(m, CAT_LAYOUT, st);
   if (!whole) TRY(reduce_wgrads(m, 7, NCONV, B, st));
-  TRY(gemm(m, m->dF8, 0, m->h7, 0, nullptr, GG(m, FC8), 0, nullptr, GG(m, FC8 + 1), m->F, 1024, B, 0, 0, ACT_NONE, st));
+  const bool d_t = ava_gemm_planes_ok(m->F, 1024, B, 0, 0) && m->lastB == B;
+  TRY(split_act(m, m->dF8, B, m->F, m->dF8_k, ava_gemm_planes_ok(B, 1024, m->F, 1, 0), m->dF8_t, d_t, GG(m, FC8 + 1), st));
+  TRY(gemm_pl(m, {m->dF8, 0, d_t ? m->dF8_t : nullptr}, {m->h7, 0, d_t ? m->h7_t : nullptr}, nullptr, GG(m, FC8), nullptr,
+              d_t ? nullptr : GG(m, FC8 + 1), m->F, 1024, B, 0, 0, ACT_NONE, st));
   return AVA_OK;
 }
 
 static int backward_part1(ava_model* m, const float* x, int B, hipStream_t st) {
   const int z = m->z;
   mark(m, -1, st);
-  TRY(gemm(m, m->dF8, 0, PP(m, FC8), 0, nullptr, m->dh7, 0, m->h7, nullptr, B, 1024, m->F, 1, 0, ACT_NONE, st));
+  TRY(gemm_pl(m, {m->dF8, 0, ava_gemm_planes_ok(B, 1024, m->F, 1, 0) ? m->dF8_k : nullptr}, {PP(m, FC8), 0, nullptr}, nullptr,
+              m->dh7, m->h7, nullptr, B, 1024, m->F, 1, 0, ACT_NONE, st));
   TRY(gemm(m, m->dh7, 0, PP(m, FC7), 0, nullptr, m->dh6, 0, m->h6, nullptr, B, 256, 1024, 1, 0, ACT_NONE, st));
   FcMidBwdArgs ba;
   ba.dh6 = m->dh6; ba.W6 = PP(m, FC6); ba.W5 = PP(m, FC5); ba.W41 = PP(m, FC41); ba.W42 = PP(m, FC42); ba.W43 = PP(m, FC43);
@@ -1054,7 +1094,10 @@
   mark(m, CAT_LATENT_LOSS, st);
   TRY(gemm(m, m->dh3, 0, PP(m, FC31), 0, nullptr, m->dh2, 0, m->h2, nullptr, B, 256, 192, 1, 0, ACT_NONE, st));
   TRY(gemm(m, m->dh2, 0, PP(m, FC2), 0, nullptr, m->dh1, 0, m->h1, nullptr, B, 1024, 256, 1, 0, ACT_NONE, st));
-  return gemm(m, m->dh1, 0, m->y7t, 0, nullptr, GG(m, FC1), 0, nullptr, GG(m, FC1 + 1), 1024, m->F, B, 0, 0, ACT_NONE, st);
+  const bool d_t = ava_gemm_planes_ok(1024, m->F, B, 0, 0) && m->lastB == B;
+  TRY(split_act(m, m->dh1, B, 1024, m->dh1_k, ava_gemm_planes_ok(B, m->F, 1024, 1, 0), m->dh1_t, d_t, GG(m, FC1 + 1), st));
+  return gemm_pl(m, {m->dh1, 0, d_t ? m->dh1_t : nullptr}, {m->y7t, 0, d_t ? m->y7t_t : nullptr}, nullptr, GG(m, FC1), nullptr,
+                 d_t ? nullptr : GG(m, FC1 + 1), 1024, m->F, B, 0, 0, ACT_NONE, st);
 }
 
 static int backward_part1b(ava_model* m, const float* x, int B, hipStream_t st) {
@@ -1062,11 +1105,8 @@
   (void)x;
   mark(m, -1, st);
   m->dy7_slabs = 1;
-  {
-    struct Mk { ava_model* m; hipStream_t st; ~Mk() { mark(m, CAT_GEMM, st); } } _mk{m, st};
-    TRY(ava_gemm_defer2(m->dh1, 0, PP(m, FC1), 0, nullptr, m->dy7, 0, nullptr, nullptr, B, m->F, 1024, 1, 0, ACT_NONE,
-                        m->dy7_ws, m->dy7_ws_bytes, st, &m->dy7_slabs));
-  }
+  TRY(gemm_pl(m, {m->dh1, 0, ava_gemm_planes_ok(B, m->F, 1024, 1, 0) ? m->dh1_k : nullptr}, {PP(m, FC1), 0, nullptr}, nullptr,
+              m->dy7, nullptr, nullptr, B, m->F, 1024, 1, 0, ACT_NONE, st, &m->dy7_slabs, m->dy7_ws, m->dy7_ws_bytes));
   const AvaGemmProblem dws[8] = {
       {m->dh7, 0, m->h6, 0, nullptr, GG(m, FC7), 0, nullptr, GG(m, FC7 + 1), 1024, 256, B, ACT_NONE},
       {m->dh6, 0, m->h5, 0, nullptr, GG(m, FC6), 0, nullptr, GG(m, FC6 + 1), 256, 64, B, ACT_NONE},
diff --git a/include/ava_hip.h b/include/ava_hip.h
--- a/include/ava_hip.h
+++ b/include/ava_hip.h
@@ -101,6 +101,13 @@
              const float* mask, float* colsum, int M, int N, int K, int a_kmajor, int b_kmajor, int act,
              void* ws, size_t ws_bytes, ava_stream_t s);
 
+size_t ava_limb_planes_bytes(int rows, int K);
+int ava_limb_split(const float* X, int ldx, int R, int C, void* planes_k, void* planes_t, float* colsum, ava_stream_t s);
+int ava_gemm_planes_used(int M, int N, int K, int a_kmajor, int b_kmajor);
+int ava_gemm_planes(const float* A, int lda, const void* a_planes, const float* B, int ldb, const void* b_planes,
+                    const float* bias, float* C, int ldc, const float* mask, float* colsum, int M, int N, int K,
+                    int a_kmajor, int b_kmajor, int act, void* ws, size_t ws_bytes, ava_stream_t s);
+
 int ava_latent_fwd(const float* mu, const float* u, const float* logd, const float* eps_w, const float* eps_d,
                    float* d, float* z, float* sums, int* status, int B, int zdim, ava_stream_t s);
 int ava_latent_bwd(const float* z, const float* dz_dec, const float* u, const float* d, const float* eps_w,
```
